# steineggerlab/folddisco

Measured on AMD Instinct MI355X. Metric: structures/sec indexed, higher is better.
Workload: dtype f32+u32; 1 GPU; Swiss-Prot scale: 542000 synthetic AFDB-shaped structures (175035960 residues, 17705019118 postings, 26085150307 value bytes) index build, PDBTrRosetta default; 1 rank(s), contiguous id ranges, per rank 1 build call(s) of <= 542000 structures: one resident index, no merge; structures=542000, structures_per_gpu=542000, residues=175035960, postings=17705019118, parallelism=shard-by-structure x1, build_calls_per_rank=1

## Files before the change

### folddisco_amd/csrc/fdgpu_api.hip

```cpp
#include <math.h>
#include <stdio.h>
#include <stdlib.h>
#include <string.h>
#include <algorithm>
#include <chrono>
#include <sys/mman.h>
#include <atomic>
#include <thread>
#include "fdgpu_internal.h"
#include <fcntl.h>
#include <unistd.h>
#include <cerrno>
#include <cstring>

#include "fd_api_common.h"
#include "fd_postings.h"

__global__ void k_uniq_flags(const uint32_t *__restrict__ keys, const uint32_t *__restrict__ ids, uint64_t n, uint8_t *__restrict__ flags) {
    uint64_t p = (uint64_t)blockIdx.x * blockDim.x + threadIdx.x;
    if (p < n) flags[p] = (p == 0 || keys[p] != keys[p - 1] || ids[p] != ids[p - 1]) ? 1 : 0;
}
__global__ void k_compact(const uint32_t *__restrict__ keys, const uint8_t *__restrict__ flags, const uint64_t *__restrict__ pos, uint64_t n,
                          uint32_t *__restrict__ out) {
    uint64_t p = (uint64_t)blockIdx.x * blockDim.x + threadIdx.x;
    if (p < n && flags[p]) out[pos[p]] = keys[p];
}
__global__ void k_gather_u64(const uint64_t *__restrict__ src, const uint64_t *__restrict__ idx, uint64_t n, uint64_t *__restrict__ dst) {
    uint64_t p = (uint64_t)blockIdx.x * blockDim.x + threadIdx.x;
    if (p < n) dst[p] = src[idx[p]];
}
void fd_launch_uniq_flags(const uint32_t *keys, const uint32_t *ids, uint64_t n, uint8_t *flags, hipStream_t st) {
    if (n) hipLaunchKernelGGL(k_uniq_flags, dim3((unsigned)((n + 255) / 256)), dim3(256), 0, st, keys, ids, n, flags);
}
void fd_launch_compact(const uint32_t *keys, const uint8_t *flags, const uint64_t *pos, uint64_t n, uint32_t *out, hipStream_t st) {
    if (n) hipLaunchKernelGGL(k_compact, dim3((unsigned)((n + 255) / 256)), dim3(256), 0, st, keys, flags, pos, n, out);
}
void fd_launch_gather_u64(const uint64_t *src, const uint64_t *idx, uint64_t n, uint64_t *dst, hipStream_t st) {
    if (n) hipLaunchKernelGGL(k_gather_u64, dim3((unsigned)((n + 255) / 256)), dim3(256), 0, st, src, idx, n, dst);
}

__global__ __launch_bounds__(256) void k_count_postings(const uint8_t *__restrict__ value, uint64_t n, unsigned long long *__restrict__ out) {
    unsigned long long acc = 0;
    for (uint64_t p = ((uint64_t)blockIdx.x * 256 + threadIdx.x) * 16; p < n; p += (uint64_t)gridDim.x * 256 * 16)
        for (uint64_t k = p; k < n && k < p + 16; ++k) acc += !(value[k] & 0x80u);
    for (int o = 32; o > 0; o >>= 1) acc += __shfl_down(acc, o);
    if ((threadIdx.x & 63) == 0 && acc) atomicAdd(out, acc);
}
hipError_t fd_count_postings(fdgpu_ctx *c, const uint8_t *value, uint64_t n, uint64_t *out) {
    unsigned long long np = 0;
    hipError_t e = hipSuccess;
    if (n) {
        e = c->ws[WS_TOTAL].ensure(64);
        if (e == hipSuccess) e = hipMemsetAsync(c->ws[WS_TOTAL].p, 0, 8, c->stream);
        if (e == hipSuccess) { hipLaunchKernelGGL(k_count_postings, dim3(2048), dim3(256), 0, c->stream, value, n, c->ws[WS_TOTAL].as<unsigned long long>()); e = hipGetLastError(); }
        if (e == hipSuccess) e = hipMemcpyAsync(&np, c->ws[WS_TOTAL].p, 8, hipMemcpyDeviceToHost, c->stream);
    }
    if (e == hipSuccess) e = hipStreamSynchronize(c->stream);
    *out = np;
    return e;
}

extern "C" const char *fdgpu_version(void) { return "folddisco_amd 0.1 (gfx950)"; }

static int fd_selfcheck(fdgpu_ctx *c) {
    const char *e = getenv("FDGPU_SELFCHECK");
    if (e && e[0] == '0') return FDGPU_OK;
    fd_hash_params p;
    memset(&p, 0, sizeof p);
    p.dist_cutoff = 20.0f; p.hash_type = FDGPU_HASH_PDBTR;
    const fd_hash_consts C = make_consts(&p);
    uint32_t *d = nullptr, h[24];
    HIPCHK(c, hipMalloc((void **)&d, sizeof h));
    fd_launch_selfcheck(C.q, d, c->stream);
    hipError_t he = hipGetLastError();
    if (he == hipSuccess) he = hipMemcpyAsync(h, d, sizeof h, hipMemcpyDeviceToHost, c->stream);
    if (he == hipSuccess) he = hipStreamSynchronize(c->stream);
    (void)hipFree(d);
    if (he != hipSuccess) { c->err = std::string("self-check launch: ") + hipGetErrorString(he); return FDGPU_EHIP; }
    static const uint32_t want[6] = {109329223u, 116878724u, 271858548u, 284511716u, 506948936u, 512052558u};
    for (int k = 0; k < 24; ++k)
        if (h[k] != want[k % 6]) {
            char b[256];
            snprintf(b, sizeof b, "self-check failed: 4CHA triad hash %d (%s evaluation) is %u, the reference's literal is %u (controller/graph.rs:71-79)", k % 6,
                     k < 6 ? "generic" : k < 12 ? "table" : k < 18 ? "speculative" : "speculative + squared-distance table", h[k], want[k % 6]);
            c->err = b;
            return FDGPU_EHIP;
        }
    int ok = 1;
    auto same = [](float a, float b) { uint32_t x, y; memcpy(&x, &a, 4); memcpy(&y, &b, 4); return x == y || (a != a && b != b); };
    for (int k = 1; k < FD_THETA_NSEG && ok; ++k) {
        float t;
        memcpy(&t, &fd_theta_thr_bits[k], 4);
        for (int u = -64; u <= 64 && ok; ++u) {
            uint32_t bits = fd_theta_thr_bits[k] + (uint32_t)u;
            float x;
            memcpy(&x, &bits, 4);
            if (!(x >= -1.0f && x <= 1.0f)) continue;
            const float a = acosf(x);
            ok = same(fd_acosf(x), a) && same(fd_sinf(a), sinf(a)) && same(fd_cosf(a), cosf(a));
        }
    }
    for (int m = 0; m < 4 && ok; ++m)
        for (int k = 1; k < FD_TOR_MAXSEG && ok; ++k)
            for (int u = -64; u <= 64 && ok; ++u) {
                uint32_t bits = fd_tor_thr_bits[m][k] + (uint32_t)u;
                float r;
                memcpy(&r, &bits, 4);
                if (!(r == r) || r > 3.0e38f) continue;
                const float y = (m & 1) ? -r : r, x = (m & 2) ? -1.0f : 1.0f;
                const float a = -atan2f(y, x);
                ok = same(-fd_atan2f(y, x), a) && same(fd_sinf(a), sinf(a)) && same(fd_cosf(a), cosf(a));
            }
    c->host_libm_matches = ok;
    if (!ok) {
        static bool warned = false;
        if (!warned) {
            warned = true;
            fprintf(stderr, "[fdgpu] warning: this host's libm (sinf/cosf/acosf/atan2f) differs from the glibc 2.35 generation the device arithmetic restates; a "
                            "reference build on this host can hash residue pairs at bin edges differently (rerun tools/gen_bin_tables.c + tools/check_libm.c)\n");
        }
    }
    return FDGPU_OK;
}
extern "C" int fdgpu_host_libm_matches(const fdgpu_ctx *c) { return c ? c->host_libm_matches : -1; }

static std::atomic<int> fd_live_contexts{0};
extern "C" void fdgpu_trim(void);
extern "C" int fdgpu_create(int device, fdgpu_ctx **out) {
    if (!out) return FDGPU_EINVAL;
    *out = nullptr;
    fdgpu_ctx *c = new (std::nothrow) fdgpu_ctx();
    if (!c) return FDGPU_ENOMEM;
    c->device = device;
    int n = 0;
    hipError_t e = hipGetDeviceCount(&n);
    if (e != hipSuccess || n <= 0 || device < 0 || device >= n) {
        c->err = e != hipSuccess ? std::string("hipGetDeviceCount: ") + hipGetErrorString(e) : "no such HIP device";
        *out = c;
        return FDGPU_EHIP;
    }
    if ((e = hipSetDevice(device)) != hipSuccess || (e = hipStreamCreate(&c->stream)) != hipSuccess) {
        c->err = std::string("hipSetDevice/hipStreamCreate: ") + hipGetErrorString(e);
        *out = c;
        return FDGPU_EHIP;
    }
    c->own_stream = true;
    c->counted = true;
    fd_live_contexts.fetch_add(1);
    if (hipMalloc((void **)&c->spec_miss, 8) == hipSuccess) (void)hipMemset(c->spec_miss, 0, 8);
    else c->spec_miss = nullptr;
    *out = c;
    return fd_selfcheck(c);
}
extern "C" int fdgpu_spec_fallbacks(fdgpu_ctx *c, uint64_t *out) { FD_LOCK(c);
    if (!c || !out) return FDGPU_EINVAL;
    *out = 0;
    if (!c->spec_miss) return FDGPU_OK;
    HIPCHK(c, hipStreamSynchronize(c->stream));
    HIPCHK(c, hipMemcpy(out, c->spec_miss, 8, hipMemcpyDeviceToHost));
    HIPCHK(c, hipMemset(c->spec_miss, 0, 8));
    return FDGPU_OK;
}
extern "C" void fdgpu_destroy(fdgpu_ctx *c) {
    if (!c) return;
    fd_lanes_destroy(c);
    if (c->spec_miss) (void)hipFree(c->spec_miss);
    for (auto &b : c->ws) b.release();
    for (auto &b : c->pool) (void)hipFree(b.p);
    for (auto e : c->event_pool) (void)hipEventDestroy(e);
    for (int k = 0; k < 16; ++k) { if (c->pin[k]) (void)hipHostFree(c->pin[k]); if (c->pin_ev[k]) (void)hipEventDestroy(c->pin_ev[k]); }
    for (int k = 0; k < 6; ++k) if (c->hbuf[k]) (void)hipHostFree(c->hbuf[k]);
    if (c->side_stream) (void)hipStreamDestroy(c->side_stream);
    if (c->own_stream && c->stream) (void)hipStreamDestroy(c->stream);
    const bool last = c->counted && fd_live_contexts.fetch_sub(1) == 1;
    delete c;
    if (last) fdgpu_trim();
}
extern "C" int fdgpu_release_workspaces(fdgpu_ctx *c) { FD_LOCK(c);
    if (!c) return FDGPU_EINVAL;
    HIPCHK(c, hipStreamSynchronize(c->stream));
    for (auto &b : c->ws) b.release();
    c->pool_drop();
    (void)hipGetLastError();
    return FDGPU_OK;
}
extern "C" int fdgpu_set_stream(fdgpu_ctx *c, void *s) { FD_LOCK(c);
    if (!c) return FDGPU_EINVAL;
    if (c->own_stream && c->stream) { (void)hipStreamSynchronize(c->stream); (void)hipStreamDestroy(c->stream); c->own_stream = false; }
    if (s) { c->stream = (hipStream_t)s; return FDGPU_OK; }
    HIPCHK(c, hipStreamCreate(&c->stream));
    c->own_stream = true;
    return FDGPU_OK;
}
extern "C" int fdgpu_synchronize(fdgpu_ctx *c) { FD_LOCK(c);
    if (!c) return FDGPU_EINVAL;
    HIPCHK(c, hipStreamSynchronize(c->stream));
    return FDGPU_OK;
}
extern "C" const char *fdgpu_last_error(const fdgpu_ctx *c) { return c ? c->err.c_str() : "null context"; }
#include <mutex>
#include <unordered_map>
namespace {
struct fd_out_blk { size_t cap; bool pinned; };
struct fd_out_pool {
    std::mutex mu;
    std::unordered_map<void *, fd_out_blk> live;
    std::vector<std::pair<fd_out_blk, void *>> idle;
    size_t idle_bytes = 0;
};
fd_out_pool &out_pool() { static fd_out_pool *p = new fd_out_pool(); return *p; }
const size_t FD_OUT_POOL_MIN = (size_t)64 << 10;
size_t fd_out_pool_cap() {
    static const size_t cap = [] { const char *e = getenv("FDGPU_OUT_POOL_MB"); return e ? (size_t)std::max(0L, atol(e)) << 20 : (size_t)256 << 20; }();
    return cap;
}
}
extern "C" void fdgpu_trim(void) {
    fd_out_pool &P = out_pool();
    std::vector<std::pair<fd_out_blk, void *>> drop;
    {
        std::lock_guard<std::mutex> lk(P.mu);
        drop.swap(P.idle);
        P.idle_bytes = 0;
    }
    for (auto &b : drop) { if (b.first.pinned) (void)hipHostFree(b.second); else free(b.second); }
}
void *fd_out_alloc(size_t bytes, bool pinned) {
    if (bytes < FD_OUT_POOL_MIN) return malloc(bytes ? bytes : 1);
    fd_out_pool &P = out_pool();
    {
        std::lock_guard<std::mutex> lk(P.mu);
        size_t best = (size_t)-1;
        for (size_t k = 0; k < P.idle.size(); ++k)
            if (P.idle[k].first.pinned == pinned && P.idle[k].first.cap >= bytes && P.idle[k].first.cap <= 2 * bytes + (1u << 20) &&
                (best == (size_t)-1 || P.idle[k].first.cap < P.idle[best].first.cap)) best = k;
        if (best != (size_t)-1) {
            void *p = P.idle[best].second;
            const fd_out_blk b = P.idle[best].first;
            P.idle.erase(P.idle.begin() + best);
            P.idle_bytes -= b.cap;
            P.live[p] = b;
            return p;
        }
    }
    const size_t cap = bytes + bytes / 4;
    void *p = nullptr;
    bool got_pinned = false;
    if (pinned && hipHostMalloc(&p, cap, hipHostMallocPortable) == hipSuccess && p) got_pinned = true;
    else { (void)hipGetLastError(); p = malloc(cap); }
    if (!p) return nullptr;
    std::lock_guard<std::mutex> lk(P.mu);
    P.live[p] = fd_out_blk{cap, got_pinned};
    return p;
}
extern "C" void fdgpu_free(void *p) {
    if (!p) return;
    fd_out_pool &P = out_pool();
    fd_out_blk b;
    {
        std::lock_guard<std::mutex> lk(P.mu);
        auto it = P.live.find(p);
        if (it == P.live.end()) { free(p); return; }
        b = it->second;
        P.live.erase(it);
        if (P.idle_bytes + b.cap <= fd_out_pool_cap()) { P.idle.emplace_back(b, p); P.idle_bytes += b.cap; return; }
    }
    if (b.pinned) (void)hipHostFree(p); else free(p);
}
extern "C" int fdgpu_enable_timing(fdgpu_ctx *c, int on) { FD_LOCK(c); if (!c) return FDGPU_EINVAL; c->timing = on != 0; return FDGPU_OK; }
extern "C" int fdgpu_last_timings(const fdgpu_ctx *c, const char **names, float *ms, uint64_t *bytes, int cap) { FD_LOCK(c);
    if (!c) return FDGPU_EINVAL;
    int n = 0;
    for (auto &t : c->timings) {
        if (n >= cap) break;
        float m = 0.f;
        if (hipEventElapsedTime(&m, t.ev0, t.ev1) != hipSuccess) m = -1.f;
        if (names) names[n] = t.name;
        if (ms) ms[n] = m;
        if (bytes) bytes[n] = t.bytes;
        ++n;
    }
    return n;
}

int fd_build_work_items(fdgpu_ctx *c, fdgpu_batch *b, bool with_hash_ok) {
    std::vector<uint32_t> ws, wi;
    std::vector<uint32_t> ro(b->n_struct + 1);
    for (uint64_t s = 0; s <= b->n_struct; ++s) ro[s] = (uint32_t)b->h_res_off[s];
    for (uint64_t s = 0; s < b->n_struct; ++s) {
        uint64_t R = b->h_res_off[s + 1] - b->h_res_off[s];
        if (R > 65535) FAIL(c, FDGPU_ERANGE, "structure with more than 65535 residues (reference max_residue, controller/mod.rs:40)");
        for (uint64_t t = 0; t < R; t += FD_WAVE) { ws.push_back((uint32_t)s); wi.push_back((uint32_t)(b->h_res_off[s] + t)); }
    }
    if (ws.size() > 0xfffffff0ull) FAIL(c, FDGPU_ERANGE, "too many tiles in one batch");
    b->n_work = (uint32_t)ws.size();
    HIPCHK(c, hipMalloc((void **)&b->res_off, ro.size() * 4));
    HIPCHK(c, hipMalloc((void **)&b->wi_struct, std::max<size_t>(ws.size(), 1) * 4));
    HIPCHK(c, hipMalloc((void **)&b->wi_i0, std::max<size_t>(wi.size(), 1) * 4));
    HIPCHK(c, hipMemcpyAsync(b->res_off, ro.data(), ro.size() * 4, hipMemcpyHostToDevice, c->stream));
    if (!ws.empty()) {
        HIPCHK(c, hipMemcpyAsync(b->wi_struct, ws.data(), ws.size() * 4, hipMemcpyHostToDevice, c->stream));
        HIPCHK(c, hipMemcpyAsync(b->wi_i0, wi.data(), wi.size() * 4, hipMemcpyHostToDevice, c->stream));
    }
    HIPCHK(c, hipMalloc((void **)&b->hash_ok, std::max<uint64_t>(b->n_res, 1)));
    if (with_hash_ok) fd_launch_hash_ok(b->aa, b->cb_valid, b->hash_ok, b->n_res, c->stream);
    HIPCHK(c, hipGetLastError());
    HIPCHK(c, hipStreamSynchronize(c->stream));
    return FDGPU_OK;
}

extern "C" int fdgpu_batch_upload(fdgpu_ctx *c, const fd_batch_desc *h, fdgpu_batch **out) { FD_LOCK(c);
    if (!c || !h || !out || !h->res_off || (h->n_struct && (!h->n_xyz || !h->ca_xyz || !h->cb_xyz || !h->aa))) return FDGPU_EINVAL;
    *out = nullptr;
    if (h->n_struct >= 0xffffffffull) FAIL(c, FDGPU_ERANGE, "too many structures in one batch");
    uint64_t R = h->res_off[h->n_struct];
    if (R >= 0xffffffffull) FAIL(c, FDGPU_ERANGE, "more than 2^32 residues in one batch");
    fdgpu_batch *b = new (std::nothrow) fdgpu_batch();
    if (!b) return FDGPU_ENOMEM;
    b->ctx = c; b->owns = true; b->n_struct = h->n_struct; b->n_res = R;
    b->h_res_off.assign(h->res_off, h->res_off + h->n_struct + 1);
    size_t rb = std::max<uint64_t>(R, 1);
    int rc = FDGPU_OK;
    auto up = [&](void **d, const void *src, size_t bytes) -> int {
        HIPCHK(c, hipMalloc(d, std::max<size_t>(bytes, 4)));
        if (bytes) HIPCHK(c, hipMemcpyAsync(*d, src, bytes, hipMemcpyHostToDevice, c->stream));
        return FDGPU_OK;
    };
    if ((rc = up((void **)&b->n_xyz, h->n_xyz, R * 12)) || (rc = up((void **)&b->ca_xyz, h->ca_xyz, R * 12)) ||
        (rc = up((void **)&b->cb_xyz, h->cb_xyz, R * 12)) || (rc = up((void **)&b->aa, h->aa, R))) { fdgpu_batch_destroy(b); return rc; }
    if (h->cb_valid && (rc = up((void **)&b->cb_valid, h->cb_valid, R))) { fdgpu_batch_destroy(b); return rc; }
    (void)rb;
    if ((rc = fd_build_work_items(c, b))) { fdgpu_batch_destroy(b); return rc; }
    *out = b;
    return FDGPU_OK;
}

extern "C" int fdgpu_batch_wrap_device(fdgpu_ctx *c, const fd_batch_desc *d, uint64_t total_residues, fdgpu_batch **out) { FD_LOCK(c);
    if (!c || !d || !out || !d->res_off) return FDGPU_EINVAL;
    *out = nullptr;
    fdgpu_batch *b = new (std::nothrow) fdgpu_batch();
    if (!b) return FDGPU_ENOMEM;
    b->ctx = c; b->owns = false; b->n_struct = d->n_struct; b->n_res = total_residues;
    b->n_xyz = (float *)d->n_xyz; b->ca_xyz = (float *)d->ca_xyz; b->cb_xyz = (float *)d->cb_xyz;
    b->aa = (uint8_t *)d->aa; b->cb_valid = (uint8_t *)d->cb_valid;
    b->h_res_off.resize(d->n_struct + 1);
    hipError_t e = hipMemcpy(b->h_res_off.data(), d->res_off, (d->n_struct + 1) * 8, hipMemcpyDeviceToHost);
    if (e != hipSuccess) { c->err = std::string("wrap_device: ") + hipGetErrorString(e); delete b; return FDGPU_EHIP; }
    if (b->h_res_off[d->n_struct] != total_residues) { c->err = "wrap_device: res_off[n] != total_residues"; delete b; return FDGPU_EINVAL; }
    int rc = fd_build_work_items(c, b);
    if (rc) { fdgpu_batch_destroy(b); return rc; }
    *out = b;
    return FDGPU_OK;
}

extern "C" void fdgpu_batch_destroy(fdgpu_batch *b) {
    if (!b) return;
    if (b->owns) { (void)hipFree(b->n_xyz); (void)hipFree(b->ca_xyz); (void)hipFree(b->cb_xyz); (void)hipFree(b->aa); (void)hipFree(b->cb_valid); }
    (void)hipFree(b->hash_ok); (void)hipFree(b->res_off); (void)hipFree(b->wi_struct); (void)hipFree(b->wi_i0);
    delete b;
}
extern "C" uint64_t fdgpu_batch_num_structures(const fdgpu_batch *b) { return b ? b->n_struct : 0; }
extern "C" uint64_t fdgpu_batch_num_residues(const fdgpu_batch *b) { return b ? b->n_res : 0; }

bool fd_hash_type_supported(uint32_t t) { return t <= 8u; }
fd_hash_consts make_consts_bins(const fd_hash_params *p, uint32_t nbd_req, uint32_t nba_req, bool either_zero_defaults) {
    const uint32_t type = p->hash_type;
    uint32_t cap_d = 16, def_d = 16, cap_a = 4, def_a = 4;
    if (type == FD_HASH_PDBMOTIF) { cap_d = 32; def_d = 18; cap_a = 32; def_a = 9; }
    else if (type == FD_HASH_PDBMOTIF_SINCOS) { cap_d = 16; def_d = 8; cap_a = 16; def_a = 3; }
    else if (type == FD_HASH_FD_ANGLE) { cap_d = 8; def_d = 8; cap_a = 32; def_a = 32; }
    else if (type == FD_HASH_FD_DIST) { cap_d = 32; def_d = 32; cap_a = 16; def_a = 16; }
    else if (type == FD_HASH_TRROSETTA) { cap_d = 8; def_d = 8; cap_a = 4; def_a = 3; }
    else if (type == FD_HASH_PPF || type == FD_HASH_TERTIARY) { cap_d = 16; def_d = 8; cap_a = 8; def_a = 3; }
    else if (type == FD_HASH_HYBRID) { cap_d = 16; def_d = 16; cap_a = 4; def_a = 4; }
    const bool dflt = either_zero_defaults && (nbd_req == 0 || nba_req == 0);
    float nd = (dflt || nbd_req == 0) ? (float)def_d : (nbd_req > cap_d ? (float)cap_d : (float)nbd_req);
    float na = (dflt || nba_req == 0) ? (float)def_a : (nba_req > cap_a ? (float)cap_a : (float)nba_req);
    fd_hash_consts C;
    C.seg_mul = 1; C.seg_cfg = 0;
    const float PI_F = 3.14159274f;
    float a_min = -1.0f, a_max = 1.0f;
    if (type == FD_HASH_PDBMOTIF) { a_min = 0.0f; a_max = 180.0f; }
    else if (type == FD_HASH_FD_ANGLE || type == FD_HASH_FD_DIST) { a_min = -PI_F; a_max = PI_F; }
    volatile float cont_d = (20.0f - 2.0f) / (nd - 1.0f);
    volatile float cont_a = (a_max - a_min) / (na - 1.0f);
    float n180 = type == FD_HASH_FD_ANGLE ? fminf(na, 32.0f) : fminf(na, 8.0f);
    volatile float cont_t = (PI_F - 0.0f) / (n180 - 1.0f);
    C.q.dist_disc = 1.0f / cont_d;
    C.q.ang_disc = 1.0f / cont_a;
    C.q.ang2_disc = 1.0f / cont_t;
    C.q.type = type;
    float cut = p->dist_cutoff;
    float d2 = cut * cut;
    while (sqrtf(d2) > cut) d2 = nextafterf(d2, 0.0f);
    while (sqrtf(nextafterf(d2, INFINITY)) <= cut) d2 = nextafterf(d2, INFINITY);
    C.d2_max = d2;
    const char *ex = getenv("FDGPU_EXACT");
    const bool exact_only = ex && ex[0] == '1';
    C.use_tab = (type == FD_HASH_PDBTR && na == 4.0f) ? (exact_only ? 1 : 2) : 0;
    const char *dt = getenv("FDGPU_DTAB");
    if (C.use_tab == 2 && nd == 16.0f && !(dt && dt[0] == '0')) C.use_tab = 3;
    C.spec_miss = nullptr;
    return C;
}

fd_hash_consts make_consts(const fd_hash_params *p) { return make_consts_bins(p, p->nbin_dist, p->nbin_angle, true); }
fd_hash_consts fd_make_consts(const fd_hash_params *p) { return make_consts(p); }
uint32_t fd_num_bin_configs(const fd_hash_params *p) { return p->n_multiple_bins ? p->n_multiple_bins : 1u; }
fd_hash_consts fd_make_consts_cfg(const fd_hash_params *p, uint32_t k) {
    if (!p->n_multiple_bins) return make_consts(p);
    return make_consts_bins(p, p->multiple_bins[k][0], p->multiple_bins[k][1], false);
}
bool fd_multiple_bins_valid(const fd_hash_params *p) {
    if (p->n_multiple_bins > FDGPU_MAX_MULTIPLE_BINS) return false;
    for (uint32_t k = 0; k < p->n_multiple_bins; ++k)
        if (p->multiple_bins[k][0] == 0 || p->multiple_bins[k][1] == 0) return false;
    return true;
}

int d2h_u64(fdgpu_ctx *c, const uint64_t *dev, uint64_t *host) {
    HIPCHK(c, hipMemcpyAsync(host, dev, 8, hipMemcpyDeviceToHost, c->stream));
    HIPCHK(c, hipStreamSynchronize(c->stream));
    return FDGPU_OK;
}

static int count_and_scan(fdgpu_ctx *c, const fdgpu_batch *b, const fd_hash_consts &C, uint64_t *P, bool unordered = false) {
    uint64_t S = b->n_struct;
    HIPCHK(c, c->ws[WS_COUNTS].ensure((S + 1) * 4));
    HIPCHK(c, c->ws[WS_CURSOR].ensure((S + 1) * 4));
    HIPCHK(c, c->ws[WS_SEGOFF].ensure((S + 2) * 8));
    HIPCHK(c, c->ws[WS_SCANTMP].ensure(fd_scan_tmp_elems(std::max<uint64_t>(S, b->n_res)) * 8 + 64));
    HIPCHK(c, c->ws[WS_TOTAL].ensure(64));
    HIPCHK(c, hipMemsetAsync(c->ws[WS_COUNTS].p, 0, (S + 1) * 4, c->stream));
    HIPCHK(c, hipMemsetAsync(c->ws[WS_CURSOR].p, 0, (S + 1) * 4, c->stream));
    {
        StageTimer t(c, "pair_count", b->n_res * 13);
        if (unordered) fd_launch_pair_count2(b->view(), C, c->ws[WS_COUNTS].as<uint32_t>(), c->stream);
        else fd_launch_pair_count(b->view(), C, c->ws[WS_COUNTS].as<uint32_t>(), c->stream);
    }
    {
        StageTimer t(c, "segment_scan", S * 12);
        fd_exclusive_scan<uint32_t>(c->ws[WS_COUNTS].as<uint32_t>(), S, c->ws[WS_SEGOFF].as<uint64_t>(), c->ws[WS_SCANTMP].as<uint64_t>(),
                                    c->ws[WS_TOTAL].as<uint64_t>(), c->stream);
    }
    HIPCHK(c, hipGetLastError());
    return d2h_u64(c, c->ws[WS_TOTAL].as<uint64_t>(), P);
}

static int ensure_sort_ws(fdgpu_ctx *c, uint64_t P, size_t id_bytes = 4) {
    size_t kb = std::max<uint64_t>(P, 1) * 4, ib = std::max<uint64_t>(P, 1) * id_bytes + 16;
    if (kb > c->ws[WS_KEYS_A].cap + ((size_t)1 << 30) || kb > c->ws[WS_KEYS_B].cap + ((size_t)1 << 30)) c->pool_drop();
    HIPCHK(c, c->ws[WS_KEYS_A].ensure(kb));
    HIPCHK(c, c->ws[WS_IDS_A].ensure(ib));
    HIPCHK(c, c->ws[WS_KEYS_B].ensure(kb));
    HIPCHK(c, c->ws[WS_IDS_B].ensure(ib));
    HIPCHK(c, c->ws[WS_GHIST].ensure((size_t)256 * std::max<uint32_t>(fd_rs_num_tiles(P), 1) * 4));
    HIPCHK(c, c->ws[WS_TOT].ensure((256 + (size_t)(fd_rs_num_tiles(P) / 128 + 2) * 256) * 8));
    return FDGPU_OK;
}

int sort_pairs(fdgpu_ctx *c, uint32_t *ka, uint32_t *va, uint32_t *kb, uint32_t *vb, uint64_t n, int key_bits) {
    return fd_radix_sort_pairs(ka, va, kb, vb, n, key_bits, c->ws[WS_GHIST].as<uint32_t>(), c->ws[WS_TOT].as<uint64_t>(), c->stream, c);
}

extern "C" int fdgpu_hash_batch(fdgpu_ctx *c, const fdgpu_batch *b, const fd_hash_params *p, int sort_dedup, uint32_t **hashes,
                                uint64_t **hash_off) { FD_LOCK(c);
    if (!c || !b || !p || !hashes || !hash_off) return FDGPU_EINVAL;
    *hashes = nullptr; *hash_off = nullptr;
    if (p->n_multiple_bins) FAIL(c, FDGPU_EINVAL, "hash_batch: multiple_bins is honoured by the index build and the query calls only");
    if (!fd_hash_type_supported(p->hash_type)) FAIL(c, FDGPU_EINVAL, "hash_type: only the encodings over the (d_CA, d_CB, theta, tau1, tau2) descriptor are built (0, 1, 3, 7, 8)");
    reset_timings(c);
    fd_hash_consts C = make_consts(p);
    uint64_t S = b->n_struct, R = b->n_res;
    uint64_t *h_off = (uint64_t *)malloc((S + 1) * 8);
    if (!h_off) return FDGPU_ENOMEM;
    hipStream_t st = c->stream;
    if (!sort_dedup) {
        HIPCHK(c, c->ws[WS_MISC0].ensure((R + 1) * 4));
        HIPCHK(c, c->ws[WS_MISC1].ensure((R + 2) * 8));
        HIPCHK(c, c->ws[WS_SCANTMP].ensure(fd_scan_tmp_elems(std::max<uint64_t>(S, R)) * 8 + 64));
        HIPCHK(c, c->ws[WS_TOTAL].ensure(64));
        HIPCHK(c, hipMemsetAsync(c->ws[WS_MISC0].p, 0, (R + 1) * 4, st));
        fd_launch_row_count(b->view(), C, c->ws[WS_MISC0].as<uint32_t>(), p->dist_cutoff, st);
        fd_exclusive_scan<uint32_t>(c->ws[WS_MISC0].as<uint32_t>(), R, c->ws[WS_MISC1].as<uint64_t>(), c->ws[WS_SCANTMP].as<uint64_t>(),
                                    c->ws[WS_TOTAL].as<uint64_t>(), st);
        HIPCHK(c, hipGetLastError());
        uint64_t P = 0;
        int rc = d2h_u64(c, c->ws[WS_TOTAL].as<uint64_t>(), &P);
        if (rc) { free(h_off); return rc; }
        HIPCHK(c, c->ws[WS_KEYS_A].ensure(std::max<uint64_t>(P, 1) * 4));
        fd_launch_row_emit(b->view(), C, c->ws[WS_MISC1].as<uint64_t>(), c->ws[WS_KEYS_A].as<uint32_t>(), p->dist_cutoff, nullptr, 0u, st);
        HIPCHK(c, hipGetLastError());
        uint32_t *h = (uint32_t *)malloc(std::max<uint64_t>(P, 1) * 4);
        std::vector<uint64_t> row_off(R + 1);
        if (!h) { free(h_off); return FDGPU_ENOMEM; }
        HIPCHK(c, hipMemcpyAsync(h, c->ws[WS_KEYS_A].p, P * 4, hipMemcpyDeviceToHost, st));
        HIPCHK(c, hipMemcpyAsync(row_off.data(), c->ws[WS_MISC1].p, (R + 1) * 8, hipMemcpyDeviceToHost, st));
        HIPCHK(c, hipStreamSynchronize(st));
        for (uint64_t s = 0; s <= S; ++s) h_off[s] = row_off[b->h_res_off[s]];
        *hashes = h; *hash_off = h_off;
        return FDGPU_OK;
    }
    if (fd_own_descriptor(p->hash_type)) { free(h_off); FAIL(c, FDGPU_EINVAL, "hash_batch: this encoding is served in the reference's raw order only (sort_dedup = 0)"); }
    uint64_t P = 0;
    int rc = count_and_scan(c, b, C, &P);
    if (rc) { free(h_off); return rc; }
    if (P >= 0xffffffffull) { free(h_off); FAIL(c, FDGPU_ERANGE, "more than 2^32 residue pairs in one batch; split the batch"); }
    if ((rc = ensure_sort_ws(c, P))) { free(h_off); return rc; }
    uint32_t *ka = c->ws[WS_KEYS_A].as<uint32_t>(), *ia = c->ws[WS_IDS_A].as<uint32_t>();
    uint32_t *kb = c->ws[WS_KEYS_B].as<uint32_t>(), *ib = c->ws[WS_IDS_B].as<uint32_t>();
    fd_launch_pair_emit(b->view(), C, c->ws[WS_SEGOFF].as<uint64_t>(), c->ws[WS_CURSOR].as<uint32_t>(), ka, ia, 0u, st);
    int cur = sort_pairs(c, ka, ia, kb, ib, P, 32);
    uint32_t *k1 = cur ? kb : ka, *i1 = cur ? ib : ia, *k2 = cur ? ka : kb, *i2 = cur ? ia : ib;
    int id_bits = 1;
    while (id_bits < 32 && (1ull << id_bits) < std::max<uint64_t>(S, 2)) ++id_bits;
    int cur2 = sort_pairs(c, i1, k1, i2, k2, P, id_bits);
    uint32_t *ids_s = cur2 ? i2 : i1, *keys_s = cur2 ? k2 : k1, *spare = cur2 ? k1 : k2;
    HIPCHK(c, c->ws[WS_MISC0].ensure(std::max<uint64_t>(P, 1)));
    HIPCHK(c, c->ws[WS_MISC1].ensure((P + 2) * 8));
    HIPCHK(c, c->ws[WS_SCANTMP].ensure(fd_scan_tmp_elems(std::max<uint64_t>(P, S)) * 8 + 64));
    fd_launch_uniq_flags(keys_s, ids_s, P, c->ws[WS_MISC0].as<uint8_t>(), st);
    fd_exclusive_scan<uint8_t>(c->ws[WS_MISC0].as<uint8_t>(), P, c->ws[WS_MISC1].as<uint64_t>(), c->ws[WS_SCANTMP].as<uint64_t>(),
                               c->ws[WS_TOTAL].as<uint64_t>(), st);
    fd_launch_compact(keys_s, c->ws[WS_MISC0].as<uint8_t>(), c->ws[WS_MISC1].as<uint64_t>(), P, spare, st);
    HIPCHK(c, c->ws[WS_MISC2].ensure((S + 2) * 8));
    fd_launch_gather_u64(c->ws[WS_MISC1].as<uint64_t>(), c->ws[WS_SEGOFF].as<uint64_t>(), S + 1, c->ws[WS_MISC2].as<uint64_t>(), st);
    HIPCHK(c, hipGetLastError());
    uint64_t U = 0;
    if ((rc = d2h_u64(c, c->ws[WS_TOTAL].as<uint64_t>(), &U))) { free(h_off); return rc; }
    uint32_t *h = (uint32_t *)malloc(std::max<uint64_t>(U, 1) * 4);
    if (!h) { free(h_off); return FDGPU_ENOMEM; }
    HIPCHK(c, hipMemcpyAsync(h, spare, U * 4, hipMemcpyDeviceToHost, st));
    HIPCHK(c, hipMemcpyAsync(h_off, c->ws[WS_MISC2].p, (S + 1) * 8, hipMemcpyDeviceToHost, st));
    HIPCHK(c, hipStreamSynchronize(st));
    *hashes = h; *hash_off = h_off;
    return FDGPU_OK;
}

extern "C" int fdgpu_hash_batch_rows(fdgpu_ctx *c, const fdgpu_batch *b, const fd_hash_params *p, uint32_t **hashes, uint32_t **partner, uint64_t **row_off) { FD_LOCK(c);
    if (!c || !b || !p || !hashes || !partner || !row_off) return FDGPU_EINVAL;
    *hashes = nullptr; *partner = nullptr; *row_off = nullptr;
    if (p->n_multiple_bins) FAIL(c, FDGPU_EINVAL, "hash_batch_rows: multiple_bins is honoured by the index build and the query calls only");
    if (!fd_hash_type_supported(p->hash_type)) FAIL(c, FDGPU_EINVAL, "hash_type: unknown encoding");
    reset_timings(c);
    const fd_hash_consts C = make_consts(p);
    const uint64_t R = b->n_res;
    hipStream_t st = c->stream;
    HIPCHK(c, c->ws[WS_MISC0].ensure((R + 1) * 4));
    HIPCHK(c, c->ws[WS_MISC1].ensure((R + 2) * 8));
    HIPCHK(c, c->ws[WS_SCANTMP].ensure(fd_scan_tmp_elems(std::max<uint64_t>(b->n_struct, R)) * 8 + 64));
    HIPCHK(c, c->ws[WS_TOTAL].ensure(64));
    HIPCHK(c, hipMemsetAsync(c->ws[WS_MISC0].p, 0, (R + 1) * 4, st));
    fd_launch_row_count(b->view(), C, c->ws[WS_MISC0].as<uint32_t>(), p->dist_cutoff, st);
    fd_exclusive_scan<uint32_t>(c->ws[WS_MISC0].as<uint32_t>(), R, c->ws[WS_MISC1].as<uint64_t>(), c->ws[WS_SCANTMP].as<uint64_t>(),
                                c->ws[WS_TOTAL].as<uint64_t>(), st);
    HIPCHK(c, hipGetLastError());
    uint64_t P = 0;
    int rc = d2h_u64(c, c->ws[WS_TOTAL].as<uint64_t>(), &P);
    if (rc) return rc;
    HIPCHK(c, c->ws[WS_KEYS_A].ensure(std::max<uint64_t>(P, 1) * 4));
    HIPCHK(c, c->ws[WS_IDS_A].ensure(std::max<uint64_t>(P, 1) * 4));
    fd_launch_row_emit(b->view(), C, c->ws[WS_MISC1].as<uint64_t>(), c->ws[WS_KEYS_A].as<uint32_t>(), p->dist_cutoff, c->ws[WS_IDS_A].as<uint32_t>(), 0u, st, 1);
    HIPCHK(c, hipGetLastError());
    uint32_t *h = (uint32_t *)malloc(std::max<uint64_t>(P, 1) * 4), *pj = (uint32_t *)malloc(std::max<uint64_t>(P, 1) * 4);
    uint64_t *ro = (uint64_t *)malloc((R + 1) * 8);
    if (!h || !pj || !ro) { free(h); free(pj); free(ro); return FDGPU_ENOMEM; }
    hipError_t e = hipMemcpyAsync(h, c->ws[WS_KEYS_A].p, P * 4, hipMemcpyDeviceToHost, st);
    if (e == hipSuccess) e = hipMemcpyAsync(pj, c->ws[WS_IDS_A].p, P * 4, hipMemcpyDeviceToHost, st);
    if (e == hipSuccess) e = hipMemcpyAsync(ro, c->ws[WS_MISC1].p, (R + 1) * 8, hipMemcpyDeviceToHost, st);
    if (e == hipSuccess) e = hipStreamSynchronize(st);
    if (e != hipSuccess) { free(h); free(pj); free(ro); c->err = std::string("hash_batch_rows: ") + hipGetErrorString(e); return FDGPU_EHIP; }
    *hashes = h; *partner = pj; *row_off = ro;
    return FDGPU_OK;
}

hipError_t fd_index_block(fdgpu_ctx *pool, size_t bytes, void **p, size_t *cap) {
    if (!pool) return hipMalloc(p, bytes);
    hipError_t e;
    *p = pool->pool_alloc(bytes, &e);
    *cap = pool->last_cap;
    return e;
}
int fd_index_new(fdgpu_ctx *c, bool pooled, uint64_t H, uint64_t value_len, bool with_last, fdgpu_index **out) {
    *out = nullptr;
    fdgpu_index *ix = new (std::nothrow) fdgpu_index();
    if (!ix) FAIL(c, FDGPU_ENOMEM, "index alloc: out of memory");
    ix->ctx = pooled ? c : nullptr; ix->n_hashes = H;
    hipError_t e = hipSuccess;
    if (value_len != FD_VALUE_LATER) { ix->value_len = value_len; e = fd_index_block(ix->ctx, value_len + FD_VALUE_SLACK, (void **)&ix->value, &ix->cap_value); }
    if (e == hipSuccess) e = fd_index_block(ix->ctx, std::max<uint64_t>(H, 1) * 4, (void **)&ix->hashes, &ix->cap_hashes);
    if (e == hipSuccess) e = fd_index_block(ix->ctx, (H + 1) * 8, (void **)&ix->offsets, &ix->cap_offsets);
    if (e == hipSuccess && with_last) e = fd_index_block(ix->ctx, std::max<uint64_t>(H, 1) * 4, (void **)&ix->last_ids, &ix->cap_last);
    if (e != hipSuccess) { c->err = std::string("index alloc: ") + hipGetErrorString(e); fdgpu_index_destroy(ix); return FDGPU_EHIP; }
    *out = ix;
    return FDGPU_OK;
}
__global__ void k_ix_order(const uint8_t *__restrict__ sel, const uint8_t *__restrict__ is_long, const uint64_t *__restrict__ sel_pre,
                           const uint64_t *__restrict__ long_pre, uint64_t H, uint32_t *__restrict__ order, uint32_t *__restrict__ place) {
    const uint64_t t = (uint64_t)blockIdx.x * blockDim.x + threadIdx.x;
    if (t >= H || (sel && !sel[t])) return;
    const uint64_t n_long = long_pre[H];
    const uint64_t g = is_long[t] ? long_pre[t] : n_long + ((sel ? sel_pre[t] : t) - long_pre[t]);
    order[g] = (uint32_t)t;
    if (place) place[t] = (uint32_t)g;
}
void fd_order_long_first(const uint8_t *sel, const uint8_t *is_long, uint64_t H, uint64_t *sel_pre, uint64_t *long_pre, uint64_t *scan_tmp,
                         uint64_t *total_dev, uint32_t *order, uint32_t *place, hipStream_t st) {
    if (sel) fd_exclusive_scan<uint8_t>(sel, H, sel_pre, scan_tmp, total_dev, st);
    fd_exclusive_scan<uint8_t>(is_long, H, long_pre, scan_tmp, total_dev, st);
    hipLaunchKernelGGL(k_ix_order, dim3(fd_grid(H, 256)), dim3(256), 0, st, sel, is_long, sel_pre, long_pre, H, order, place);
}
extern "C" void fdgpu_index_destroy(fdgpu_index *ix) {
    if (!ix) return;
    FD_LOCK(ix->ctx);
    if (ix->ctx) {
        ix->ctx->pool_free(ix->hashes, ix->cap_hashes); ix->ctx->pool_free(ix->offsets, ix->cap_offsets); ix->ctx->pool_free(ix->value, ix->cap_value);
    } else { (void)hipFree(ix->hashes); (void)hipFree(ix->offsets); (void)hipFree(ix->value); }
    if (ix->ctx && ix->cap_last) ix->ctx->pool_free(ix->last_ids, ix->cap_last);
    else (void)hipFree(ix->last_ids);
    if (ix->penalty) (void)hipFree(ix->penalty);
    if (ix->lens) (void)hipFree(ix->lens);
    if (ix->ck_meta) (void)hipFree(ix->ck_meta);
    if (ix->ck_ent) (void)hipFree(ix->ck_ent);
    delete ix;
}
extern "C" int fdgpu_index_set_first_id(fdgpu_index *ix, uint64_t first_id) { if (!ix || first_id + ix->n_structures > 0xffffffffull) return FDGPU_EINVAL; ix->first_id = first_id; return FDGPU_OK; }
extern "C" uint64_t fdgpu_index_num_hashes(const fdgpu_index *ix) { return ix ? ix->n_hashes : 0; }
extern "C" uint64_t fdgpu_index_value_len(const fdgpu_index *ix) { return ix ? ix->value_len : 0; }
extern "C" uint64_t fdgpu_index_num_postings(const fdgpu_index *ix) { return ix ? ix->n_postings : 0; }
extern "C" uint64_t fdgpu_index_num_structures(const fdgpu_index *ix) { return ix ? ix->n_structures : 0; }

#define FDGPU_RETRY_WIDE 1000
static int encode_sorted_stream(fdgpu_ctx *c, const uint32_t *ks, const void *is, int codec, uint64_t first_id, uint64_t P, uint64_t S, fdgpu_index **out) {
    hipStream_t st = c->stream;
    const bool el6 = codec != 0;
    int rc;
    uint32_t nt = std::max<uint32_t>(fd_enc_num_tiles(P), 1);
    HIPCHK(c, c->ws[WS_TILE_B].ensure((size_t)(nt + 1) * 4));
    HIPCHK(c, c->ws[WS_TILE_H].ensure((size_t)(nt + 1) * 4));
    HIPCHK(c, c->ws[WS_TILE_P].ensure((size_t)(nt + 1) * 4));
    HIPCHK(c, c->ws[WS_TILE_BO].ensure((size_t)(nt + 2) * 8));
    HIPCHK(c, c->ws[WS_TILE_HO].ensure((size_t)(nt + 2) * 8));
    HIPCHK(c, c->ws[WS_TILE_PO].ensure((size_t)(nt + 2) * 8));
    HIPCHK(c, c->ws[WS_SCANTMP].ensure(fd_scan_tmp_elems(std::max<uint64_t>(nt, S)) * 8 + 64));
    uint64_t tot[5] = {0, 0, 0, 0, 0};
    uint64_t nt_eff = P ? fd_enc_num_tiles(P) : 0;
    {
        StageTimer t(c, "encode_sizes", P * (el6 ? 6 : 8));
        HIPCHK(c, hipMemsetAsync(c->ws[WS_TILE_B].p, 0, (size_t)(nt + 1) * 4, st));
        HIPCHK(c, hipMemsetAsync(c->ws[WS_TILE_H].p, 0, (size_t)(nt + 1) * 4, st));
        HIPCHK(c, hipMemsetAsync(c->ws[WS_TILE_P].p, 0, (size_t)(nt + 1) * 4, st));
        fd_launch_enc_sizes(ks, is, codec, (uint32_t)first_id, P, c->ws[WS_TILE_B].as<uint32_t>(), c->ws[WS_TILE_H].as<uint32_t>(), c->ws[WS_TILE_P].as<uint32_t>(),
                            c->ws[WS_SEGOFF].as<uint64_t>(), S, c->ws[WS_MISC3].as<uint64_t>() + 8, st);
        uint64_t *totd = c->ws[WS_MISC3].as<uint64_t>();
        fd_exclusive_scan<uint32_t>(c->ws[WS_TILE_B].as<uint32_t>(), nt_eff, c->ws[WS_TILE_BO].as<uint64_t>(), c->ws[WS_SCANTMP].as<uint64_t>(), totd + 0, st);
        fd_exclusive_scan<uint32_t>(c->ws[WS_TILE_H].as<uint32_t>(), nt_eff, c->ws[WS_TILE_HO].as<uint64_t>(), c->ws[WS_SCANTMP].as<uint64_t>(), totd + 1, st);
        fd_exclusive_scan<uint32_t>(c->ws[WS_TILE_P].as<uint32_t>(), nt_eff, c->ws[WS_TILE_PO].as<uint64_t>(), c->ws[WS_SCANTMP].as<uint64_t>(), totd + 2, st);
    }
    HIPCHK(c, hipGetLastError());
    HIPCHK(c, hipMemcpyAsync(tot, c->ws[WS_MISC3].p, 40, hipMemcpyDeviceToHost, st));
    HIPCHK(c, hipStreamSynchronize(st));
    if (tot[4]) FAIL(c, FDGPU_ERANGE, "index build: one (residue-pair bucket, key digit) group holds 2^32 keys or more; build the shard in several calls and merge");
    if (el6 && tot[3]) return FDGPU_RETRY_WIDE;
    fdgpu_index *ix = nullptr;
    if ((rc = fd_index_new(c, true, tot[1], tot[0], true, &ix))) return rc;
    ix->n_postings = tot[2]; ix->n_structures = S; ix->first_id = first_id;
    {
        StageTimer t(c, "encode_write", P * (el6 ? 6 : 8) + ix->value_len + ix->n_hashes * 12);
        fd_launch_enc_write(ks, is, codec, (uint32_t)first_id, P, c->ws[WS_TILE_BO].as<uint64_t>(), c->ws[WS_TILE_HO].as<uint64_t>(), ix->value, ix->hashes, ix->offsets,
                            ix->last_ids, c->ws[WS_MISC3].as<uint64_t>(), ix->n_hashes, c->ws[WS_MISC3].as<uint64_t>() + 8, st);
    }
    const hipError_t e = hipGetLastError();
    if (e != hipSuccess) { c->err = std::string("encode launch: ") + hipGetErrorString(e); fdgpu_index_destroy(ix); return FDGPU_EHIP; }
    *out = ix;
    return FDGPU_OK;
}

static int index_build_impl(fdgpu_ctx *c, const fdgpu_batch *b, const fd_hash_params *p, uint64_t first_id, fdgpu_index **out, bool force32) {
    if (!c || !b || !p || !out) return FDGPU_EINVAL;
    *out = nullptr;
    if (!fd_hash_type_supported(p->hash_type)) FAIL(c, FDGPU_EINVAL, "hash_type: only the encodings over the (d_CA, d_CB, theta, tau1, tau2) descriptor are built (0, 1, 3, 7, 8)");
    reset_timings(c);
    if (first_id + b->n_struct > 0xffffffffull) FAIL(c, FDGPU_ERANGE, "structure ids exceed 32 bits");
    if (!fd_multiple_bins_valid(p)) FAIL(c, FDGPU_EINVAL, "multiple_bins: at most 8 (dist, angle) bin pairs, no zero counts");
    const uint32_t n_cfg = fd_num_bin_configs(p);
    fd_hash_consts C = fd_make_consts_cfg(p, 0);
    C.spec_miss = c->spec_miss;
    hipStream_t st = c->stream;
    uint64_t S = b->n_struct, P = 0;
    HIPCHK(c, c->ws[WS_FRAMES].ensure(std::max<uint64_t>(b->n_res, 1) * sizeof(fd_frame)));
    const bool own = fd_own_descriptor(p->hash_type);
    if (own && n_cfg > 1) FAIL(c, FDGPU_EINVAL, "multiple_bins is built for the encodings over the PDBTrRosetta descriptor only");
    const bool ids16 = !own && !force32 && S <= (1ull << 18);
    const bool msd_env = [] { const char *e = getenv("FDGPU_MSD"); return !(e && e[0] == '0'); }();
    const bool msd = msd_env && !own && !force32 && S <= (1ull << 24) && n_cfg == 1 && p->hash_type == FDGPU_HASH_PDBTR && S > 0;
    const bool el6 = ids16 || msd;
    const int codec = msd ? 2 : ids16 ? 1 : 0;
    const uint32_t NB = 40;
    fd_batch_view V = b->view();
    HIPCHK(c, c->ws[WS_MISC3].ensure(512));
    HIPCHK(c, hipMemsetAsync(c->ws[WS_MISC3].p, 0, 64, st));
    C.wide_flag = c->ws[WS_MISC3].as<unsigned long long>() + 3;
    if (msd) {
        HIPCHK(c, c->ws[WS_CA_PERM].ensure(std::max<uint64_t>(b->n_res, 1) * 12));
        HIPCHK(c, c->ws[WS_OK_PERM].ensure(std::max<uint64_t>(b->n_res, 1)));
        HIPCHK(c, c->ws[WS_AA_PERM].ensure(std::max<uint64_t>(b->n_res, 1)));
        StageTimer t(c, "frames", b->n_res * (37 + sizeof(fd_frame) + 14));
        fd_launch_frames_perm(V, c->ws[WS_FRAMES].p, c->ws[WS_CA_PERM].as<float>(), c->ws[WS_OK_PERM].as<uint8_t>(), c->ws[WS_AA_PERM].as<uint8_t>(), C.wide_flag, st);
        V.ca_xyz = c->ws[WS_CA_PERM].as<float>(); V.hash_ok = c->ws[WS_OK_PERM].as<uint8_t>(); V.aa = c->ws[WS_AA_PERM].as<uint8_t>();
        V.n_xyz = nullptr; V.cb_xyz = nullptr;
    } else {
        StageTimer t(c, "frames", b->n_res * (37 + sizeof(fd_frame)));
        fd_launch_frames(b->view(), b->n_res, c->ws[WS_FRAMES].p, st);
    }
    uint64_t P1 = 0;
    int rc;
    if (own) {
        const uint64_t R = b->n_res;
        HIPCHK(c, c->ws[WS_MISC0].ensure((R + 1) * 4));
        HIPCHK(c, c->ws[WS_MISC1].ensure((R + 2) * 8));
        HIPCHK(c, c->ws[WS_SCANTMP].ensure(fd_scan_tmp_elems(std::max<uint64_t>(R, S)) * 8 + 64));
        HIPCHK(c, c->ws[WS_TOTAL].ensure(64));
        HIPCHK(c, hipMemsetAsync(c->ws[WS_MISC0].p, 0, (R + 1) * 4, st));
        {
            StageTimer t(c, "pair_count", R * 37);
            fd_launch_row_count(b->view(), C, c->ws[WS_MISC0].as<uint32_t>(), p->dist_cutoff, st);
            fd_exclusive_scan<uint32_t>(c->ws[WS_MISC0].as<uint32_t>(), R, c->ws[WS_MISC1].as<uint64_t>(), c->ws[WS_SCANTMP].as<uint64_t>(),
                                        c->ws[WS_TOTAL].as<uint64_t>(), st);
        }
        HIPCHK(c, hipGetLastError());
        rc = d2h_u64(c, c->ws[WS_TOTAL].as<uint64_t>(), &P1);
    } else if (msd) {
        const uint64_t NS = NB * S;
        HIPCHK(c, c->ws[WS_COUNTS].ensure((NS + 1) * 4));
        HIPCHK(c, c->ws[WS_CURSOR].ensure((NS + 1) * 4));
        HIPCHK(c, c->ws[WS_SEGOFF].ensure((NS + 2) * 8));
        HIPCHK(c, c->ws[WS_SCANTMP].ensure(fd_scan_tmp_elems(std::max<uint64_t>(NS, b->n_res)) * 8 + 64));
        HIPCHK(c, c->ws[WS_TOTAL].ensure(64));
        HIPCHK(c, hipMemsetAsync(c->ws[WS_COUNTS].p, 0, (NS + 1) * 4, st));
        HIPCHK(c, hipMemsetAsync(c->ws[WS_CURSOR].p, 0, (NS + 1) * 4, st));
        {
            StageTimer t(c, "pair_count", b->n_res * 14);
            fd_launch_pair_count_msd(V, C, c->ws[WS_COUNTS].as<uint32_t>(), st);
        }
        {
            StageTimer t(c, "segment_scan", NS * 12);
            fd_exclusive_scan<uint32_t>(c->ws[WS_COUNTS].as<uint32_t>(), NS, c->ws[WS_SEGOFF].as<uint64_t>(), c->ws[WS_SCANTMP].as<uint64_t>(),
                                        c->ws[WS_TOTAL].as<uint64_t>(), st);
        }
        HIPCHK(c, hipGetLastError());
        rc = d2h_u64(c, c->ws[WS_TOTAL].as<uint64_t>(), &P1);
        uint64_t odd = 0;
        if (!rc) rc = d2h_u64(c, (const uint64_t *)C.wide_flag, &odd);
        if (!rc && odd) return FDGPU_RETRY_WIDE;
    } else {
        rc = count_and_scan(c, b, C, &P1, true);
    }
    if (rc) return rc;
    P = P1 * n_cfg;
    if (P >= 0xffffffffull && !msd) FAIL(c, FDGPU_ERANGE, "more than 2^32 residue pairs in one build call; split the shard");
    if (P >= (1ull << 35)) FAIL(c, FDGPU_ERANGE, "more than 2^35 residue pairs in one build call; split the shard");
    if ((rc = ensure_sort_ws(c, P, el6 ? 2 : 4))) return rc;
    uint32_t *ka = c->ws[WS_KEYS_A].as<uint32_t>(), *kb = c->ws[WS_KEYS_B].as<uint32_t>();
    void *ia = c->ws[WS_IDS_A].p, *ib = c->ws[WS_IDS_B].p;
    {
        StageTimer t(c, "pair_emit", b->n_res * 37 + P * (el6 ? 6 : 8));
        if (own) fd_launch_row_emit(b->view(), C, c->ws[WS_MISC1].as<uint64_t>(), ka, p->dist_cutoff, (uint32_t *)ia, (uint32_t)first_id, st);
        else if (msd) fd_launch_pair_emit_msd(V, c->ws[WS_FRAMES].p, C, c->ws[WS_SEGOFF].as<uint64_t>(), c->ws[WS_CURSOR].as<uint32_t>(), ka, (uint16_t *)ia, st);
        else for (uint32_t k = 0; k < n_cfg; ++k) {
            fd_hash_consts Ck = fd_make_consts_cfg(p, k);
            Ck.spec_miss = C.spec_miss; Ck.wide_flag = C.wide_flag; Ck.seg_mul = n_cfg; Ck.seg_cfg = k;
            if (k) HIPCHK(c, hipMemsetAsync(c->ws[WS_CURSOR].p, 0, (S + 1) * 4, st));
            fd_launch_pair_emit2(b->view(), c->ws[WS_FRAMES].p, Ck, c->ws[WS_SEGOFF].as<uint64_t>(), c->ws[WS_CURSOR].as<uint32_t>(), ka, ia, ids16,
                                 (uint32_t)first_id, st);
        }
    }
    int cur;
    if (msd) {
        static const fd_rs_digit digits[3] = {{0, 24}, {1, 0}, {1, 8}};
        HIPCHK(c, c->ws[WS_GHIST].ensure((size_t)256 * fd_rs_seg_num_tiles(P, NB) * 4));
        HIPCHK(c, c->ws[WS_TOT].ensure(fd_rs_seg_tot_words(P, NB) * 8));
        HIPCHK(c, c->ws[WS_SEG_TAB].ensure(fd_rs_seg_tab_bytes(P, NB)));
        cur = fd_radix_sort_pairs16_seg(ka, (uint16_t *)ia, kb, (uint16_t *)ib, P, c->ws[WS_SEGOFF].as<uint64_t>(), S, NB, digits, 3, c->ws[WS_GHIST].as<uint32_t>(),
                                        c->ws[WS_TOT].as<uint64_t>(), c->ws[WS_SEG_TAB].p, st, c, c->ws[WS_MISC3].as<unsigned long long>() + 4);
    } else if (ids16) cur = fd_radix_sort_pairs16(ka, (uint16_t *)ia, kb, (uint16_t *)ib, P, 32, c->ws[WS_GHIST].as<uint32_t>(), c->ws[WS_TOT].as<uint64_t>(), st, c);
    else cur = sort_pairs(c, ka, (uint32_t *)ia, kb, (uint32_t *)ib, P, 32);
    const uint32_t *ks = cur ? kb : ka;
    const void *is = cur ? ib : ia;
    return encode_sorted_stream(c, ks, is, codec, first_id, P, S, out);
}

extern "C" int fdgpu_index_build(fdgpu_ctx *c, const fdgpu_batch *b, const fd_hash_params *p, uint64_t first_id, fdgpu_index **out) { FD_LOCK(c);
    const char *e32 = getenv("FDGPU_IDS32");
    int rc = index_build_impl(c, b, p, first_id, out, e32 && e32[0] == '1');
    if (rc == FDGPU_RETRY_WIDE) rc = index_build_impl(c, b, p, first_id, out, true);
    return rc;
}

extern "C" int fdgpu_debug_encode_stream(fdgpu_ctx *c, const uint32_t *hashes, const uint32_t *ids, uint64_t n, fdgpu_index **out) { FD_LOCK(c);
    if (!c || !out || (n && (!hashes || !ids))) return FDGPU_EINVAL;
    *out = nullptr;
    if (n >= 0xffffffffull) FAIL(c, FDGPU_ERANGE, "encode_stream: 2^32 elements or more");
    uint64_t S = 0;
    for (uint64_t p = 0; p < n; ++p) {
        if (p && (hashes[p - 1] > hashes[p] || (hashes[p - 1] == hashes[p] && ids[p - 1] > ids[p]))) FAIL(c, FDGPU_EINVAL, "encode_stream: the stream is not sorted by (hash, id)");
        S = std::max<uint64_t>(S, (uint64_t)ids[p] + 1);
    }
    reset_timings(c);
    hipStream_t st = c->stream;
    HIPCHK(c, c->ws[WS_MISC3].ensure(512));
    HIPCHK(c, hipMemsetAsync(c->ws[WS_MISC3].p, 0, 64, st));
    HIPCHK(c, c->ws[WS_KEYS_A].ensure(std::max<uint64_t>(n, 1) * 4));
    HIPCHK(c, c->ws[WS_IDS_A].ensure(std::max<uint64_t>(n, 1) * 4));
    if (n) {
        HIPCHK(c, hipMemcpyAsync(c->ws[WS_KEYS_A].p, hashes, n * 4, hipMemcpyHostToDevice, st));
        HIPCHK(c, hipMemcpyAsync(c->ws[WS_IDS_A].p, ids, n * 4, hipMemcpyHostToDevice, st));
    }
    return encode_sorted_stream(c, c->ws[WS_KEYS_A].as<uint32_t>(), c->ws[WS_IDS_A].p, 0, 0, n, S, out);
}

#define FD_PIN_SLOTS 16
#define FD_PIN_BYTES ((size_t)16 << 20)
hipError_t fd_d2h_big(fdgpu_ctx *c, void *dst, const void *src, size_t bytes) {
    if (bytes < 4 * FD_PIN_BYTES) return bytes ? hipMemcpyAsync(dst, src, bytes, hipMemcpyDeviceToHost, c->stream) : hipSuccess;
    for (int k = 0; k < FD_PIN_SLOTS; ++k) {
        hipError_t e = hipSuccess;
        if (!c->pin[k]) e = hipHostMalloc(&c->pin[k], FD_PIN_BYTES, hipHostMallocDefault);
        if (e == hipSuccess && !c->pin_ev[k]) e = hipEventCreateWithFlags(&c->pin_ev[k], hipEventDisableTiming);
        if (e != hipSuccess) return hipMemcpyAsync(dst, src, bytes, hipMemcpyDeviceToHost, c->stream);
    }
    {
        const uintptr_t a = ((uintptr_t)dst + 0x1fffff) & ~(uintptr_t)0x1fffff, b = ((uintptr_t)dst + bytes) & ~(uintptr_t)0x1fffff;
        if (b > a) (void)madvise((void *)a, b - a, MADV_HUGEPAGE);
    }
    const size_t n_chunks = (bytes + FD_PIN_BYTES - 1) / FD_PIN_BYTES;
    std::vector<std::thread> drain(FD_PIN_SLOTS);
    hipError_t err = hipSuccess;
    const int dev = c->device;
    for (size_t i = 0; i < n_chunks && err == hipSuccess; ++i) {
        const int k = (int)(i % FD_PIN_SLOTS);
        if (drain[k].joinable()) drain[k].join();
        const size_t off = i * FD_PIN_BYTES, n = std::min(FD_PIN_BYTES, bytes - off);
        err = hipMemcpyAsync(c->pin[k], (const uint8_t *)src + off, n, hipMemcpyDeviceToHost, c->stream);
        if (err == hipSuccess) err = hipEventRecord(c->pin_ev[k], c->stream);
        if (err != hipSuccess) break;
        void *pin = c->pin[k];
        hipEvent_t ev = c->pin_ev[k];
        drain[k] = std::thread([=]() { (void)hipSetDevice(dev); (void)hipEventSynchronize(ev); memcpy((uint8_t *)dst + off, pin, n); });
    }
    for (auto &t : drain) if (t.joinable()) t.join();
    return err;
}

extern "C" int fdgpu_index_export(fdgpu_ctx *c, const fdgpu_index *ix, uint8_t **value, uint64_t *value_len, uint32_t **hashes,
                                  uint64_t **offsets, uint64_t *n_hashes) { FD_LOCK(c);
    if (!c || !ix || !value || !value_len || !hashes || !offsets || !n_hashes) return FDGPU_EINVAL;
    uint8_t *v = (uint8_t *)malloc(std::max<uint64_t>(ix->value_len, 1));
    uint32_t *h = (uint32_t *)malloc(std::max<uint64_t>(ix->n_hashes, 1) * 4);
    uint64_t *o = (uint64_t *)malloc((ix->n_hashes + 1) * 8);
    if (!v || !h || !o) { free(v); free(h); free(o); return FDGPU_ENOMEM; }
    hipError_t e = fd_d2h_big(c, v, ix->value, ix->value_len);
    if (e == hipSuccess) e = fd_d2h_big(c, h, ix->hashes, ix->n_hashes * 4);
    if (e == hipSuccess) e = fd_d2h_big(c, o, ix->offsets, (ix->n_hashes + 1) * 8);
    if (e == hipSuccess) e = hipStreamSynchronize(c->stream);
    if (e != hipSuccess) { free(v); free(h); free(o); c->err = std::string("index export: ") + hipGetErrorString(e); return FDGPU_EHIP; }
    *value = v; *value_len = ix->value_len; *hashes = h; *offsets = o; *n_hashes = ix->n_hashes;
    return FDGPU_OK;
}

extern "C" int fdgpu_index_load(fdgpu_ctx *c, const uint32_t *hashes, const uint64_t *offsets, uint64_t H, const uint8_t *value,
                                uint64_t vlen, uint64_t n_structures, fdgpu_index **out) { FD_LOCK(c);
    if (!c || !out || (H && (!hashes || !offsets)) || (vlen && !value)) return FDGPU_EINVAL;
    *out = nullptr;
    fdgpu_index *ix = nullptr;
    int rc = fd_index_new(c, false, H, vlen, false, &ix);
    if (rc) return rc;
    ix->n_structures = n_structures;
    hipError_t e = hipSuccess;
    uint64_t zero = 0;
    if ((vlen && (e = hipMemcpyAsync(ix->value, value, vlen, hipMemcpyHostToDevice, c->stream)) != hipSuccess) ||
        (H && (e = hipMemcpyAsync(ix->hashes, hashes, H * 4, hipMemcpyHostToDevice, c->stream)) != hipSuccess) ||
        (e = hipMemcpyAsync(ix->offsets, H ? offsets : &zero, (H + 1) * 8, hipMemcpyHostToDevice, c->stream)) != hipSuccess ||
        (e = hipStreamSynchronize(c->stream)) != hipSuccess) {
        c->err = std::string("index load: ") + hipGetErrorString(e);
        fdgpu_index_destroy(ix);
        return FDGPU_EHIP;
    }
    if ((e = fd_count_postings(c, ix->value, vlen, &ix->n_postings)) != hipSuccess) {
        (void)hipGetLastError();
        c->err = std::string("index load: counting the postings: ") + hipGetErrorString(e);
        fdgpu_index_destroy(ix);
        return FDGPU_EHIP;
    }
    *out = ix;
    return FDGPU_OK;
}

hipError_t fd_d2h_to_file(fdgpu_ctx *c, int fd, uint64_t file_off, const void *src, size_t bytes, std::atomic<int> *io_err) {
    if (!bytes) return hipSuccess;
    for (int k = 0; k < FD_PIN_SLOTS; ++k) {
        hipError_t e = hipSuccess;
        if (!c->pin[k]) e = hipHostMalloc(&c->pin[k], FD_PIN_BYTES, hipHostMallocDefault);
        if (e == hipSuccess && !c->pin_ev[k]) e = hipEventCreateWithFlags(&c->pin_ev[k], hipEventDisableTiming);
        if (e != hipSuccess) return e;
    }
    const size_t n_chunks = (bytes + FD_PIN_BYTES - 1) / FD_PIN_BYTES;
    std::vector<std::thread> drain(FD_PIN_SLOTS);
    hipError_t err = hipSuccess;
    const int dev = c->device;
    for (size_t i = 0; i < n_chunks && err == hipSuccess; ++i) {
        const int k = (int)(i % FD_PIN_SLOTS);
        if (drain[k].joinable()) drain[k].join();
        const size_t off = i * FD_PIN_BYTES, n = std::min(FD_PIN_BYTES, bytes - off);
        err = hipMemcpyAsync(c->pin[k], (const uint8_t *)src + off, n, hipMemcpyDeviceToHost, c->stream);
        if (err == hipSuccess) err = hipEventRecord(c->pin_ev[k], c->stream);
        if (err != hipSuccess) break;
        const uint8_t *pin = (const uint8_t *)c->pin[k];
        hipEvent_t ev = c->pin_ev[k];
        drain[k] = std::thread([=]() {
            (void)hipSetDevice(dev);
            if (hipEventSynchronize(ev) != hipSuccess) { int z = 0; io_err->compare_exchange_strong(z, EIO); return; }
            size_t done = 0;
            while (done < n) {
                const ssize_t w = pwrite(fd, pin + done, n - done, (off_t)(file_off + off + done));
                if (w < 0) { if (errno == EINTR) continue; int z = 0; io_err->compare_exchange_strong(z, errno ? errno : EIO); return; }
                done += (size_t)w;
            }
        });
    }
    for (auto &t : drain) if (t.joinable()) t.join();
    return err;
}

extern "C" int fdgpu_reserve_staging(fdgpu_ctx *c) { FD_LOCK(c);
    if (!c) return FDGPU_EINVAL;
    for (int k = 0; k < FD_PIN_SLOTS; ++k) {
        if (!c->pin[k]) HIPCHK(c, hipHostMalloc(&c->pin[k], FD_PIN_BYTES, hipHostMallocDefault));
        if (!c->pin_ev[k]) HIPCHK(c, hipEventCreateWithFlags(&c->pin_ev[k], hipEventDisableTiming));
    }
    return FDGPU_OK;
}

extern "C" int fdgpu_index_save(fdgpu_ctx *c, const fdgpu_index *ix, const char *prefix) { FD_LOCK(c);
    if (!c || !ix || !prefix) return FDGPU_EINVAL;
    const std::string p(prefix);
    const uint64_t H = ix->n_hashes;
    std::atomic<int> io_err{0};
    hipError_t e = hipSuccess;
    const int fv = open(p.c_str(), O_WRONLY | O_CREAT | O_TRUNC, 0644);
    const int fo = fv >= 0 ? open((p + ".offset").c_str(), O_WRONLY | O_CREAT | O_TRUNC, 0644) : -1;
    if (fv < 0 || fo < 0) { if (fv >= 0) close(fv); FAIL(c, FDGPU_EINVAL, "index save: cannot write " + p); }
    if (pwrite(fo, &H, 8, 0) != 8) io_err = errno ? errno : EIO;
    const bool trace = getenv("FDGPU_TRACE") != nullptr;
    const auto t0 = std::chrono::steady_clock::now();
    auto ms = [&]() { return std::chrono::duration<double, std::milli>(std::chrono::steady_clock::now() - t0).count(); };
    if (trace) {
        for (int k = 0; k < FD_PIN_SLOTS && e == hipSuccess; ++k) if (!c->pin[k]) e = hipHostMalloc(&c->pin[k], FD_PIN_BYTES, hipHostMallocDefault);
        fprintf(stderr, "[index_save] staging slots page-locked at %.3f ms\n", ms());
    }
    if (e == hipSuccess) e = fd_d2h_to_file(c, fv, 0, ix->value, ix->value_len, &io_err);
    if (trace) fprintf(stderr, "[index_save] %llu value bytes streamed at %.3f ms\n", (unsigned long long)ix->value_len, ms());
    if (e == hipSuccess) e = fd_d2h_to_file(c, fo, 8, ix->hashes, H * 4, &io_err);
    if (e == hipSuccess) e = fd_d2h_to_file(c, fo, 8 + H * 4, ix->offsets, (H + 1) * 8, &io_err);
    if (e == hipSuccess) e = hipStreamSynchronize(c->stream);
    if (trace) fprintf(stderr, "[index_save] offset file streamed at %.3f ms\n", ms());
    if (close(fv) != 0 && !io_err) io_err = errno ? errno : EIO;
    if (close(fo) != 0 && !io_err) io_err = errno ? errno : EIO;
    if (trace) fprintf(stderr, "[index_save] files closed at %.3f ms\n", ms());
    if (e != hipSuccess) { c->err = std::string("index save: ") + hipGetErrorString(e); return FDGPU_EHIP; }
    if (io_err) FAIL(c, FDGPU_EINVAL, "index save: cannot write " + p + " (" + strerror(io_err) + ")");
    return FDGPU_OK;
}

__global__ void k_debug_libm(int op, const float *__restrict__ a, const float *__restrict__ b, float *__restrict__ out, uint64_t n) {
    uint64_t k = (uint64_t)blockIdx.x * blockDim.x + threadIdx.x;
    if (k >= n) return;
    float x = a[k], s, c;
    switch (op) {
        case 0: fdd_sincosf(x, &s, &c); out[k] = s; break;
        case 1: fdd_sincosf(x, &s, &c); out[k] = c; break;
        case 2: out[k] = fdd_acosf(x); break;
        case 3: out[k] = fdd_atanf(x); break;
        default: out[k] = fdd_atan2f(x, b[k]); break;
    }
}
extern "C" int fdgpu_debug_libm(fdgpu_ctx *c, int op, const float *a, const float *b, float *out, uint64_t n) { FD_LOCK(c);
    if (!c || !a || !out || (op == 4 && !b) || op < 0 || op > 4) return FDGPU_EINVAL;
    if (!n) return FDGPU_OK;
    hipStream_t st = c->stream;
    HIPCHK(c, c->ws[WS_MISC0].ensure(n * 4));
    HIPCHK(c, c->ws[WS_MISC1].ensure(n * 4));
    HIPCHK(c, c->ws[WS_MISC2].ensure(n * 4));
    HIPCHK(c, hipMemcpyAsync(c->ws[WS_MISC0].p, a, n * 4, hipMemcpyHostToDevice, st));
    if (b) HIPCHK(c, hipMemcpyAsync(c->ws[WS_MISC1].p, b, n * 4, hipMemcpyHostToDevice, st));
    hipLaunchKernelGGL(k_debug_libm, dim3((unsigned)((n + 255) / 256)), dim3(256), 0, st, op, c->ws[WS_MISC0].as<float>(),
                       c->ws[WS_MISC1].as<float>(), c->ws[WS_MISC2].as<float>(), n);
    HIPCHK(c, hipGetLastError());
    HIPCHK(c, hipMemcpyAsync(out, c->ws[WS_MISC2].p, n * 4, hipMemcpyDeviceToHost, st));
    HIPCHK(c, hipStreamSynchronize(st));
    return FDGPU_OK;
}
```

### folddisco_amd/csrc/fdgpu_internal.h

```cpp
#pragma once
#include <hip/hip_runtime.h>
#include <stdint.h>
#include <functional>
#include <mutex>
#include <string>
#include <vector>
#include "../../include/fdgpu.h"
#include "../../include/fdgpu_debug.h"
#include "fd_device.h"
#include "fd_geom_other.h"
#include "fd_retrieve_host.h"

#include <condition_variable>
#include <thread>
struct fd_host_pool {
    std::vector<std::thread> th;
    std::mutex mu;
    std::condition_variable cv, cv_done;
    const std::function<void()> *job = nullptr;
    uint64_t gen = 0;
    unsigned want = 0, taken = 0, active = 0;
    bool stop = false;
    void loop() {
        uint64_t seen = 0;
        for (;;) {
            const std::function<void()> *f = nullptr;
            {
                std::unique_lock<std::mutex> lk(mu);
                cv.wait(lk, [&] { return stop || (gen != seen && taken < want); });
                if (stop) return;
                seen = gen; ++taken; f = job;
            }
            (*f)();
            {
                std::lock_guard<std::mutex> lk(mu);
                --active;
            }
            cv_done.notify_one();
        }
    }
    void run(unsigned n, const std::function<void()> &f) {
        if (n <= 1) { f(); return; }
        const unsigned helpers = n - 1;
        {
            std::lock_guard<std::mutex> lk(mu);
            while (th.size() < helpers) th.emplace_back([this] { loop(); });
            job = &f; want = helpers; taken = 0; active = helpers; ++gen;
        }
        cv.notify_all();
        f();
        std::unique_lock<std::mutex> lk(mu);
        cv_done.wait(lk, [&] { return active == 0; });
        job = nullptr;
    }
    ~fd_host_pool() {
        {
            std::lock_guard<std::mutex> lk(mu);
            stop = true;
        }
        cv.notify_all();
        for (auto &t : th) t.join();
    }
};

struct fd_devbuf {
    void *p = nullptr;
    size_t cap = 0;
    hipError_t ensure(size_t bytes) {
        if (bytes <= cap) return hipSuccess;
        size_t want = bytes + (bytes < ((size_t)4 << 30) ? bytes / 16 : (size_t)0) + 256;
        if (cap && cap < (64u << 20) && want < cap + cap / 2) want = cap + cap / 2;
        if (p) { hipError_t e = hipFree(p); p = nullptr; cap = 0; if (e != hipSuccess) return e; }
        hipError_t e = hipMalloc(&p, want);
        if (e != hipSuccess) { p = nullptr; return e; }
        cap = want;
        return hipSuccess;
    }
    void release() { if (p) (void)hipFree(p); p = nullptr; cap = 0; }
    template <typename T> T *as() const { return reinterpret_cast<T *>(p); }
};

struct fd_timing_entry { const char *name; hipEvent_t ev0, ev1; uint64_t bytes; };

enum {
    WS_COUNTS, WS_CURSOR, WS_SEGOFF, WS_SCANTMP, WS_TOTAL, WS_KEYS_A, WS_IDS_A, WS_KEYS_B, WS_IDS_B, WS_GHIST, WS_TOT,
    WS_TILE_B, WS_TILE_H, WS_TILE_P, WS_TILE_BO, WS_TILE_HO , WS_TILE_PO, WS_MISC0, WS_MISC1, WS_MISC2, WS_MISC3, WS_MISC4, WS_MISC5, WS_FRAMES,
    WS_CQ_KIDX, WS_CQ_NSEG, WS_CQ_WSTART, WS_CQ_SEGSUM, WS_CQ_TOPN,
    WS_QT_RANGES, WS_QT_COMPACT, WS_QT_COUNT, WS_QT_AUX, WS_RS_PLAN, WS_RS_REC, WS_RS_RECRES, WS_QT_PARTIAL, WS_QT_SURV, WS_QT_ROWBITS, WS_QT_STREAM, WS_QT_STAB, WS_QT_PIECEP, WS_QT_WIN, WS_QT_HEAD, WS_RS_SPLIT, WS_MP_QSET,
    WS_CA_PERM, WS_OK_PERM, WS_AA_PERM, WS_SEG_TAB,
    WS_RS_TAB, WS_RS_SEG, WS_RS_OUT, WS_RS_RES, WS_RS_KX, WS_RS_KY, WS_RS_KOFF, WS_RS_SOL, WS_RS_CNT, WS_RS_GQ, WS_MP_ACT, WS_MP_Q,
    WS_SG_TAB , WS_SG_TAB_B, WS_SG_PAIRS, WS_SG_CURSOR,
    WS_SG_NB_PART , WS_SG_NB_OUT ,
    WS_COUNT
};

struct fdgpu_ctx {
    int device = 0;
    hipStream_t stream = nullptr;
    bool own_stream = false;
    std::string err;
    uint32_t last_retrieve_path = 0;
    uint32_t last_count_path = 0;
    fd_devbuf ws[WS_COUNT];
    bool timing = false;
    mutable std::recursive_mutex mu;
    int host_libm_matches = -1;
    unsigned long long *spec_miss = nullptr;
    std::vector<fd_timing_entry> timings;
    std::vector<hipEvent_t> event_pool;
    size_t event_used = 0;
    hipStream_t side_stream = nullptr;
    void *hbuf[6] = {nullptr, nullptr, nullptr, nullptr, nullptr, nullptr};
    size_t hbuf_cap[6] = {0, 0, 0, 0, 0, 0};
    void *host_pinned(int k, size_t bytes) {
        if (hbuf_cap[k] >= bytes) return hbuf[k];
        if (hbuf[k]) (void)hipHostFree(hbuf[k]);
        hbuf[k] = nullptr; hbuf_cap[k] = 0;
        const size_t want = bytes + bytes / 4 + 4096;
        if (hipHostMalloc(&hbuf[k], want, hipHostMallocDefault) != hipSuccess) { hbuf[k] = nullptr; return nullptr; }
        hbuf_cap[k] = want;
        return hbuf[k];
    }
    void *pin[16] = {};
    hipEvent_t pin_ev[16] = {};
    struct pooled { void *p; size_t cap; };
    std::vector<pooled> pool;
    void *pool_alloc(size_t bytes, hipError_t *err) {
        *err = hipSuccess;
        size_t best = (size_t)-1;
        for (size_t k = 0; k < pool.size(); ++k)
            if (pool[k].cap >= bytes && pool[k].cap <= bytes + bytes / 4 + 4096 && (best == (size_t)-1 || pool[k].cap < pool[best].cap)) best = k;
        if (best != (size_t)-1) { void *p = pool[best].p; last_cap = pool[best].cap; pool.erase(pool.begin() + best); return p; }
        void *p = nullptr;
        size_t want = bytes + bytes / 32 + 256;
        *err = hipMalloc(&p, want);
        if (*err != hipSuccess) {
            pool_drop();
            (void)hipGetLastError();
            *err = hipMalloc(&p, want);
            if (*err != hipSuccess) return nullptr;
        }
        last_cap = want;
        return p;
    }
    void pool_drop() { for (auto &b : pool) (void)hipFree(b.p); pool.clear(); }
    void pool_free(void *p, size_t cap) {
        if (!p) return;
        if (pool.size() >= 96) { (void)hipFree(p); return; }
        pool.push_back({p, cap});
    }
    size_t last_cap = 0;
    bool counted = false;
    const void *mp_bintab_at = nullptr; size_t mp_bintab_cap = 0;
    fd_host_pool host_pool;
    bool is_lane = false;
    unsigned small_par(unsigned n) const { return is_lane ? 1u : std::min(n, std::max(1u, std::thread::hardware_concurrency())); }
    void *lanes = nullptr;
};
void fd_lanes_destroy(fdgpu_ctx *c);

static inline hipEvent_t fd_next_event(fdgpu_ctx *c) {
    if (c->event_used == c->event_pool.size()) {
        hipEvent_t e;
        if (hipEventCreate(&e) != hipSuccess) return nullptr;
        c->event_pool.push_back(e);
    }
    return c->event_pool[c->event_used++];
}
struct StageTimer {
    fdgpu_ctx *c;
    size_t idx = (size_t)-1;
    StageTimer(fdgpu_ctx *ctx, const char *name, uint64_t bytes) : c(ctx) {
        if (!c || !c->timing) return;
        fd_timing_entry t;
        t.name = name; t.bytes = bytes; t.ev0 = fd_next_event(c); t.ev1 = fd_next_event(c);
        if (!t.ev0 || !t.ev1) return;
        (void)hipEventRecord(t.ev0, c->stream);
        c->timings.push_back(t);
        idx = c->timings.size() - 1;
    }
    ~StageTimer() { if (idx != (size_t)-1) (void)hipEventRecord(c->timings[idx].ev1, c->stream); }
};

#define FD_LOCK(c) std::unique_lock<std::recursive_mutex> _fd_lk; if (c) { _fd_lk = std::unique_lock<std::recursive_mutex>((c)->mu); (void)hipSetDevice((c)->device); }

struct fdgpu_batch {
    fdgpu_ctx *ctx = nullptr;
    bool owns = false;
    uint64_t n_struct = 0, n_res = 0;
    uint32_t n_work = 0;
    float *n_xyz = nullptr, *ca_xyz = nullptr, *cb_xyz = nullptr;
    uint8_t *aa = nullptr, *cb_valid = nullptr, *hash_ok = nullptr;
    uint32_t *res_off = nullptr, *wi_struct = nullptr, *wi_i0 = nullptr;
    std::vector<uint64_t> h_res_off;
    fd_batch_view view() const {
        fd_batch_view v;
        v.n_xyz = n_xyz; v.ca_xyz = ca_xyz; v.cb_xyz = cb_xyz; v.aa = aa; v.hash_ok = hash_ok; v.res_off = res_off;
        v.wi_struct = wi_struct; v.wi_i0 = wi_i0; v.n_struct = (uint32_t)n_struct; v.n_work = n_work;
        return v;
    }
};

int fd_build_work_items(fdgpu_ctx *c, fdgpu_batch *b, bool with_hash_ok = true);

#include <atomic>
static inline uint64_t fd_next_index_uid() { static std::atomic<uint64_t> n{1}; return n.fetch_add(1); }
struct fdgpu_index {
    fdgpu_ctx *ctx = nullptr;
    uint64_t n_hashes = 0, value_len = 0, n_postings = 0, n_structures = 0, first_id = 0;
    uint32_t *hashes = nullptr;
    uint64_t *offsets = nullptr;
    uint8_t *value = nullptr;
    mutable uint32_t *last_ids = nullptr;
    size_t cap_hashes = 0, cap_offsets = 0, cap_value = 0, cap_last = 0;
    mutable uint32_t *lens = nullptr;
    mutable std::mutex lens_mu;
    uint64_t uid = fd_next_index_uid();
    float *penalty = nullptr;
    mutable unsigned long long *ck_meta = nullptr;
    mutable void *ck_ent = nullptr;
    mutable uint64_t ck_n = 0, ck_first = 0, ck_S = 0;
    mutable bool ck_failed = false;
    mutable uint32_t ck_fail_skips = 0;
};

#define FD_VALUE_LATER (~0ull)
int fd_index_new(fdgpu_ctx *c, bool pooled, uint64_t H, uint64_t value_len, bool with_last, fdgpu_index **out);
hipError_t fd_index_block(fdgpu_ctx *pool, size_t bytes, void **p, size_t *cap);
int fd_index_last_ids(fdgpu_ctx *c, const fdgpu_index *ix);
hipError_t fd_count_postings(fdgpu_ctx *c, const uint8_t *value, uint64_t n, uint64_t *out);
static inline unsigned fd_grid(uint64_t n, uint64_t per) { return (unsigned)((n + per - 1) / per); }

#define FD_IXERR_DAMAGED 1u
#define FD_IXERR_LONG 2u
#define FD_LONG_LIST_BYTES 16384u
void fd_order_long_first(const uint8_t *sel, const uint8_t *is_long, uint64_t H, uint64_t *sel_pre, uint64_t *long_pre, uint64_t *scan_tmp,
                         uint64_t *total_dev, uint32_t *order, uint32_t *place, hipStream_t st);
static inline int fd_index_last_ids_staged(fdgpu_ctx *c, const fdgpu_index *ix, const char *stage) {
    if (ix->last_ids || !ix->n_hashes) return FDGPU_OK;
    StageTimer t(c, stage, ix->value_len + ix->n_hashes * 12);
    return fd_index_last_ids(c, ix);
}
struct fd_rows_dev { const uint32_t *val; const uint64_t *row_off; uint64_t n; };
int fd_rows_device(fdgpu_ctx *c, const fdgpu_index *ix, uint64_t id_lo, uint64_t id_hi, const char *what, fd_rows_dev *out);
static inline int fd_index_op_failed(fdgpu_ctx *c, int rc, fdgpu_index *const *made, size_t n = 1) {
    (void)hipStreamSynchronize(c->stream);
    for (size_t k = 0; k < n; ++k) fdgpu_index_destroy(made[k]);
    return rc;
}

struct fd_cq_dev_out {
    bool got = false, overflow = false; const void *recs = nullptr; const void *state = nullptr; uint32_t top_n = 0, cap = 0;
    std::vector<uint32_t> counts;
    const std::function<void()> *while_running = nullptr;
    uint32_t head_n = 0;
    const fd_count_rec *head = nullptr;
};
int fd_count_query_batch_impl(fdgpu_ctx *c, const fdgpu_index *ix, uint64_t n_queries, const uint64_t *q_off, const uint32_t *q_hash,
                              const uint32_t *q_node, const uint32_t *q_edge_j, const float *q_idf, const float *penalty, uint32_t top_n,
                              fd_count_rec **out, uint64_t **out_off, bool allow_dense, fd_cq_dev_out *dev, int64_t known_segments = -1,
                              const long long *known_kidx = nullptr, const uint64_t *known_len = nullptr);
int fd_posting_lengths_dev(fdgpu_ctx *c, const fdgpu_index *ix, const uint32_t *q_hash, uint64_t nq, uint64_t **dev_lengths);
uint64_t fd_maps_hashes(uint64_t n_queries, const fd_query_map *const *qms, std::vector<uint32_t> &h);
int fd_count_query_maps_len(fdgpu_ctx *c, const fdgpu_index *ix, uint64_t n_queries, const fd_query_map *const *qms, const uint64_t *len,
                            const uint64_t *primary_len, const float *penalty, float total_structures, uint32_t top_n, fd_count_rec **out,
                            uint64_t **out_off, fd_cq_dev_out *dev, const uint32_t *seg = nullptr, const long long *kidx = nullptr, bool allow_dense = true);
int fd_posting_lengths_segs(fdgpu_ctx *c, const fdgpu_index *ix, const uint32_t *q_hash, uint64_t nq, uint64_t *lengths, uint32_t *segs, long long *kidx = nullptr,
                            const uint8_t **land_out = nullptr);
int fd_count_query_maps_top_impl(fdgpu_ctx *c, const fdgpu_index *ix, uint64_t n_queries, const fd_query_map *const *qms, const float *penalty, float total_structures,
                                 uint32_t top_n, fd_count_rec **out, uint64_t **out_off, fd_cq_dev_out *dev, bool allow_dense = true);

struct fd_rb_dev_out { bool got = false; const void *recs = nullptr; const int32_t *residues = nullptr; uint64_t n_recs = 0, n_res = 0; };
int fd_retrieve_batch_dev(fdgpu_ctx *c, const fdgpu_batch *db, const uint8_t *resname_std, uint64_t n_queries, const uint32_t *cand, const uint64_t *cand_off,
                          const fd_query_map *const *qms, const fdgpu_batch *qb, const uint32_t *q_struct, const fd_hash_params *p, float ca_distance_cutoff,
                          uint32_t node_count, uint32_t partial_fit, fd_match_rec **matches, uint64_t **match_off, int32_t **residues, uint64_t **res_off, fd_rb_dev_out *dev);
hipError_t fd_d2h_to_file(fdgpu_ctx *c, int fd, uint64_t file_off, const void *src, size_t bytes, std::atomic<int> *io_err);
hipError_t fd_d2h_big(fdgpu_ctx *c, void *dst, const void *src, size_t bytes);
void *fd_out_alloc(size_t bytes, bool pinned = false);

void fd_launch_selfcheck(const fd_quant &q, uint32_t *out, hipStream_t st);
void fd_launch_hash_ok(const uint8_t *aa, const uint8_t *cb_valid, uint8_t *ok, uint64_t n, hipStream_t st);
void fd_launch_pair_count(const fd_batch_view &B, const fd_hash_consts &C, uint32_t *counts, hipStream_t st);
void fd_launch_pair_emit(const fd_batch_view &B, const fd_hash_consts &C, const uint64_t *seg_off, uint32_t *cursor, uint32_t *keys,
                         uint32_t *ids, uint32_t first_id, hipStream_t st);
void fd_launch_frames(const fd_batch_view &B, uint64_t n_res, void *frames, hipStream_t st);
void fd_launch_pair_count2(const fd_batch_view &B, const fd_hash_consts &C, uint32_t *counts, hipStream_t st);
void fd_launch_pair_emit2(const fd_batch_view &B, const void *frames, const fd_hash_consts &C, const uint64_t *seg_off, uint32_t *cursor,
                          uint32_t *keys, void *ids, bool ids16, uint32_t first_id, hipStream_t st);
int fd_radix_sort_pairs16(uint32_t *keys_a, uint16_t *vals_a, uint32_t *keys_b, uint16_t *vals_b, uint64_t n, int key_bits, uint32_t *ghist,
                          uint64_t *tot, hipStream_t st, fdgpu_ctx *timing_ctx = nullptr);
void fd_launch_frames_perm(const fd_batch_view &B, void *frames, float *ca_perm, uint8_t *ok_perm, uint8_t *aa_perm, unsigned long long *wide_flag, hipStream_t st);
void fd_launch_pair_count_msd(const fd_batch_view &B, const fd_hash_consts &C, uint32_t *counts, hipStream_t st);
void fd_launch_pair_emit_msd(const fd_batch_view &B, const void *frames, const fd_hash_consts &C, const uint64_t *seg_off, uint32_t *cursor, uint32_t *keys,
                             uint16_t *ids, hipStream_t st);
uint32_t fd_rs_seg_num_tiles(uint64_t n, uint32_t n_seg);
uint64_t fd_rs_seg_tot_words(uint64_t n, uint32_t n_seg);
size_t fd_rs_seg_tab_bytes(uint64_t n, uint32_t n_seg);
struct fd_rs_digit { uint32_t plane, shift; };
int fd_radix_sort_pairs16_seg(uint32_t *keys_a, uint16_t *vals_a, uint32_t *keys_b, uint16_t *vals_b, uint64_t n, const uint64_t *seg_off, uint64_t stride,
                              uint32_t n_seg, const fd_rs_digit *digits, int passes, uint32_t *ghist, uint64_t *tot, void *seg_tab, hipStream_t st, fdgpu_ctx *timing_ctx = nullptr,
                              unsigned long long *overflow = nullptr);
void fd_launch_row_count(const fd_batch_view &B, const fd_hash_consts &C, uint32_t *row_cnt, float cutoff, hipStream_t st);
void fd_launch_row_emit(const fd_batch_view &B, const fd_hash_consts &C, const uint64_t *row_off, uint32_t *keys, float cutoff, uint32_t *ids,
                        uint32_t first_id, hipStream_t st, int ids_partner = 0);
template <typename TIn>
void fd_exclusive_scan(const TIn *in, uint64_t n, uint64_t *out, uint64_t *chunk_tmp, uint64_t *total_dev, hipStream_t st);
uint64_t fd_scan_tmp_elems(uint64_t n);
uint32_t fd_rs_num_tiles(uint64_t n);
int fd_radix_sort_pairs(uint32_t *keys_a, uint32_t *vals_a, uint32_t *keys_b, uint32_t *vals_b, uint64_t n, int key_bits, uint32_t *ghist,
                        uint64_t *tot, hipStream_t st, fdgpu_ctx *timing_ctx = nullptr);
uint32_t fd_enc_num_tiles(uint64_t n);
void fd_launch_enc_sizes(const uint32_t *keys, const void *ids, int codec, uint32_t first_id, uint64_t n, uint32_t *tb, uint32_t *th, uint32_t *tp,
                         const uint64_t *seg_off, uint64_t S, uint64_t *bo, hipStream_t st);
void fd_launch_enc_write(const uint32_t *keys, const void *ids, int codec, uint32_t first_id, uint64_t n, const uint64_t *tbo, const uint64_t *tho,
                         uint8_t *value, uint32_t *hashes, uint64_t *offsets, uint32_t *last_ids, const uint64_t *total_bytes_dev, uint64_t H,
                         const uint64_t *bo, hipStream_t st);
void fd_launch_uniq_flags(const uint32_t *keys, const uint32_t *ids, uint64_t n, uint8_t *flags, hipStream_t st);
void fd_launch_compact(const uint32_t *keys, const uint8_t *flags, const uint64_t *pos, uint64_t n, uint32_t *out, hipStream_t st);
void fd_launch_gather_u64(const uint64_t *src, const uint64_t *idx, uint64_t n, uint64_t *dst, hipStream_t st);

struct cq_args {
    const uint32_t *hashes; const uint64_t *offsets; const uint8_t *value; uint64_t H;
    const uint32_t *q_hash; uint64_t nq;
    uint32_t *hash_bits;
    const unsigned long long *row_meta;
    uint32_t *match;
    unsigned long long *idf;
    int packed;
    uint32_t words; uint32_t first_id; uint32_t S;
};

#define QT_CELL_LOG2 11
#define QT_BINS 2048
#define QT_MAX_ROWS 1024
#define QT_MAXB 16
struct qt_state { uint32_t thr_bin, above, thr_key, count; };
struct qt_aux { uint32_t need_l2, shift2, edge, pad; };
struct qt_args {
    const uint8_t *value; const uint64_t *offsets;
    const unsigned long long *ck_meta; const uint2 *ck_ent;
    const long long *kidx;
    const unsigned long long *row_meta;
    const uint64_t *q_rows;
    const float *penalty;
    uint32_t nq, n_queries, S, first_id, NT, NC, tile_log2, plan_log2;
    uint4 *ranges;
    uint32_t *c_nid, *c_key;
    uint32_t *ccount;
    uint32_t *ghist;
    qt_state *state; qt_aux *aux;
    void *out; uint32_t cap;
    void *stream_ids; uint16_t *stream_row;
    uint2 *stream_tab;
    uint32_t *stream_used; uint32_t stream_cap;
    uint4 *pieces;
    uint32_t *piece_p;
    uint32_t *win;
    uint4 *heads;
    uint32_t win_per_row, top_n;
    uint32_t max_rows;
    const uint64_t *slices; uint32_t n_slices;
    unsigned long long *partial;
    uint32_t *g_bm, *g_rank, *g_tcount, *g_nid;
    uint32_t *g_rowbits; uint32_t g_wpr;
    const uint32_t *g_eend, *g_nend;
};
void fd_launch_ck_count(const uint64_t *offsets, uint64_t H, uint32_t NC, uint32_t *cnt, hipStream_t st);
void fd_launch_ck_fill(const uint64_t *offsets, const uint8_t *value, uint64_t H, uint32_t NC, uint32_t S, uint32_t first_id, const uint64_t *ent_off,
                       unsigned long long *meta, void *ent, hipStream_t st);
void fd_launch_qt_plan(const qt_args &A, hipStream_t st);
void fd_launch_qt_score(const qt_args &A, hipStream_t st);
void fd_launch_qt_big_score(const qt_args &A, hipStream_t st);
void fd_launch_qt_big_select(const qt_args &A, uint32_t top_n, void *sorted, hipStream_t st);
void fd_launch_qt_select(const qt_args &A, uint32_t top_n, void *sorted, hipStream_t st);
#define QT_WIN_CONT 0x80000000u
void fd_launch_qt_layout(const qt_args &A, hipStream_t st);
void fd_launch_qt_score32(const qt_args &A, hipStream_t st);

void fd_launch_index_lens(const uint64_t *offsets, const uint8_t *value, uint64_t H, uint32_t *lens, hipStream_t st);
void fd_launch_posting_lookup(const uint32_t *hashes, const uint64_t *offsets, const uint32_t *lens, uint64_t H, const uint32_t *q_hash, uint64_t nq, uint64_t *lengths,
                              uint32_t *nseg, long long *kidx, hipStream_t st);
void fd_launch_cq_plan(const cq_args &A, long long *kidx, uint32_t *nseg, hipStream_t st);
void fd_launch_cq_seg(const cq_args &A, const long long *kidx, const uint64_t *wstart, uint32_t *segsum, uint64_t n_items, bool split,
                      hipStream_t st);
void fd_launch_cq_rows_finalize(const cq_args &A, const uint64_t *q_rows, uint32_t n_queries, const uint64_t *slices, uint32_t n_slices, uint32_t *node_cnt,
                                uint32_t *edge_cnt, uint8_t *flags, uint64_t max_rows_per_query, hipStream_t st);

struct mp_query_dev {
    uint32_t qh_off, n_hashes;
    uint32_t aad_off, n_aad;
    uint32_t aa1_mask, aa2_mask;
    int use_prefilter;
    float ca_window;
    uint32_t qs_off, qs_mask;
};
#define MP_QH_LDS 1024
#define MP_SUBQ_STRIDE 16u
struct mp_args {
    fd_batch_view B;
    fd_hash_consts C;
    float cutoff;
    const uint32_t *cand; uint32_t n_cand;
    const uint32_t *wi_cand; const uint32_t *wi_i0; const uint32_t *wi_query; uint32_t n_work;
    const uint32_t *wi_j0; uint32_t j_span;
    const mp_query_dev *qtab;
    const uint32_t *qset;
    const uint8_t *resname_std;
    uint32_t aa1_mask, aa2_mask;
    int use_prefilter;
    const uint32_t *q_hashes; uint32_t n_hashes;
    const uint32_t *aad_start;
    const float *aad_dist; const uint32_t *aad_qi; uint32_t n_aad;
    const uint32_t *iv_start; const float2 *iv;
    const uint32_t *iv_grp;
    float ca_window;
    unsigned long long *n_found, *n_cands;
    const uint4 *cinfo; const uint32_t *act;
    unsigned long long *q_cnt; uint4 *chunk_hdr; uint32_t *chunk_ij; uint32_t cap_subq;
    uint32_t *res_h, *res_meta; float *res_d; uint2 *chunk_cnt; ulonglong2 *chunk_base;
    const uint32_t *bintab;
    int compact;
    fd_pair_rec *found; fd_cand_rec *cands;
    unsigned long long cap_found, cap_cands;
    uint32_t n_cfg;
    fd_quant qk[8];
    uint32_t mode;
    const uint32_t *cj_mask;
    const uint32_t *mask_off;
    uint32_t *votes; const uint64_t *vt_off; const uint32_t *vt_qs; const uint8_t *cj_comp;
    const float *sd_dist; const uint32_t *sd_qi;
};
struct fd_mp_tables {
    std::vector<uint32_t> blk; size_t o[13] = {0}; size_t nw = 0; bool want_iv = false; uint32_t j_span = 0; bool valid = false;
    const uint32_t *data = nullptr; size_t words = 0;
    bool dev_items = false; size_t o_wb = 0;
    uint64_t qset_slots = 0, qset_max_hashes = 0;
};
void fd_launch_mp_items(const uint32_t *db_res_off, const uint32_t *cand, uint32_t n_cand, const uint32_t *wbase, const uint32_t *cq, uint32_t j_span, uint32_t *wc,
                        uint32_t *wi, uint32_t *wq, uint32_t *wj, hipStream_t st, const uint8_t *aa, const uint8_t *hash_ok, const uint8_t *resname_std, int tert,
                        const struct mp_query_dev *qtab, void *cinfo , uint32_t *act );
struct fd_vote_plan {
    const uint8_t *cj_comp; uint64_t n_bits;
    const uint64_t *vt_off; const uint32_t *vt_qs; uint64_t n_counters;
    const uint64_t *row_off; const uint32_t *row_len; uint64_t n_rows;
    fd_vote_row *rows;
    const float *sd_dist; const uint32_t *sd_qi; uint64_t n_sd;
};
void fd_launch_vote_rows(const uint32_t *votes, const uint64_t *row_off, const uint32_t *row_len, uint64_t n_rows, fd_vote_row *out, hipStream_t st);
void fd_launch_match_pairs(const mp_args &A, hipStream_t st);
void fd_launch_mp_qset_build(const mp_query_dev *qtab, uint32_t n_queries, uint32_t max_hashes, const uint32_t *q_hashes, uint32_t *qset, hipStream_t st);
void fd_launch_found_key_ij(const fd_pair_rec *f, uint64_t n, uint32_t *key, uint32_t *val, hipStream_t st);
void fd_launch_found_key_slot(const fd_pair_rec *f, const uint32_t *val, uint64_t n, uint32_t *key, hipStream_t st);
void fd_launch_found_gather(const fd_pair_rec *f, const uint32_t *val, uint64_t n, fd_pair_rec *out, hipStream_t st);
void fd_launch_pack_cands(const fd_cand_rec *c, uint64_t n, uint32_t *key, uint32_t *val, hipStream_t st);
void fd_launch_kabsch(const float *x, const float *y, const uint64_t *off, uint64_t n, float *rmsd, float *rot, float *tran, hipStream_t st, uint64_t n_points = 0);
void fd_launch_metrics(const float *ref, const float *mov, const uint64_t *off, uint64_t n, const float *rot, const float *tran, const float *d0, float *out,
                       hipStream_t st, uint64_t n_points = 0);
void fd_launch_lms_qcp(const float *x, const float *y, const uint64_t *off, uint64_t n, float *rmsd, float *rot, float *tran, uint32_t *core_len,
                       uint8_t *flags, uint32_t *order, hipStream_t st);
void fd_launch_cq_compact_batch(const cq_args &A, const uint32_t *node_cnt, const uint32_t *edge_cnt, const uint8_t *flags, const uint64_t *pos,
                                const float *penalty, uint64_t total, void *out, hipStream_t st);
void fd_launch_cq_topn(const void *recs, const uint64_t *off, uint32_t n_queries, uint32_t top_n, uint32_t cap, void *out, void *state, uint32_t *ghist,
                       hipStream_t st);
void fd_launch_cq_topn_acc(const cq_args &A, const float *penalty, const uint32_t *node_cnt, const uint32_t *edge_cnt, uint32_t n_queries, uint32_t top_n,
                           uint32_t cap, void *out, void *state, uint32_t *ghist, hipStream_t st);
void fd_launch_cq_topn_dense(const cq_args &A, const uint64_t *q_rows, const float *penalty, uint32_t *keys, uint32_t n_queries, uint32_t top_n, uint32_t cap,
                             void *out, void *state, uint32_t *ghist, hipStream_t st);
void fd_launch_cq_topn_sort(const void *sel, uint32_t cap, const void *state, uint32_t n_queries, uint32_t top_n, void *out, hipStream_t st);
void fd_launch_get_entries(const uint32_t *hashes, const uint64_t *offsets, const uint8_t *value, uint64_t H, const uint32_t *q_hash, uint64_t nq,
                           const uint64_t *out_off, uint32_t *out, hipStream_t st);
struct rs_query_dev {
    uint32_t qh_off, n_hashes;
    uint32_t map_off;
    uint32_t idx_off, n_idx;
    uint32_t q_size;
    uint32_t q_res0;
    uint32_t pad;
};
struct rs_match_dev { uint32_t slot, ci, same, res_pos, prob0, prob1; float idf; uint32_t ord; };
#define RS_CNT_STRIDE 512
struct rs_args {
    const fd_pair_rec *found; const fd_cand_rec *cands;
    const uint32_t *seg_f, *seg_c, *perm_f, *perm_c;
    const uint32_t *cand, *slot_q;
    const uint32_t *order;
    uint32_t *slot_matches;
    const uint32_t *db_res_off; const float *db_ca, *db_cb, *q_ca, *q_cb;
    const rs_query_dev *qt;
    const uint32_t *hashes, *kfirst; const uint8_t *sym;
    const uint32_t *map_qi, *map_qj; const float *map_idf;
    const uint32_t *indices;
    const float *d0tab;
    uint32_t node_count;
    uint32_t node_cap;
    unsigned long long *counters;
    uint32_t *flags;
    rs_match_dev *matches; int32_t *residues; float *kx, *ky; uint64_t *koff; float *d0;
    uint32_t *gq, *gr;
    uint64_t cap_matches, cap_res, cap_prob, cap_pts;
    uint4 *sp_edges;
    uint32_t *sp_nodes;
    unsigned long long *sp_comps;
    uint4 *sp_head;
    uint2 *sp_work;
    uint4 *sp_np;
    uint32_t *sp_gq, *sp_gr;
    uint32_t *sp_big, *sp_big_n;
    const uint32_t *n_listed;
};
void fd_launch_rs_group(const fd_pair_rec *found, uint64_t nf, const fd_cand_rec *cands, uint64_t nc, uint32_t n_cand, uint32_t *cnt, uint32_t *seg, uint32_t *cur,
                        uint32_t *perm_f, uint32_t *perm_c, hipStream_t st);
void fd_launch_rs_slots(const rs_args &A, uint32_t n_cand, hipStream_t st);
void fd_launch_rs_points(const rs_args &A, uint64_t n_prob, uint64_t n_points, hipStream_t st);
void fd_launch_rs_records_dev(const void *matches, uint64_t n, const uint32_t *slot_matches, uint32_t n_cand, const uint64_t *cand_off, const uint32_t *slot_q,
                              const rs_query_dev *qt, uint32_t n_queries, uint32_t *scratch, uint64_t *match_off, uint64_t *res_off, const float *rmsd,
                              const float *rot, const float *tran, const float *met, const int32_t *residues, void *out, int32_t *out_res, hipStream_t st);
int fd_match_pairs_multi(fdgpu_ctx *c, const fdgpu_batch *db, const uint8_t *resname_std, uint64_t n_queries, const fd_match_query *qs,
                         const uint32_t *cand, const uint64_t *cand_off, const fd_hash_params *p, fd_pair_rec **found, uint64_t *n_found,
                         fd_cand_rec **cands, uint64_t *n_cands, uint32_t mode = 3, const uint32_t *cj_mask = nullptr,
                         const uint32_t *mask_off = nullptr, uint64_t mask_words = 0, uint32_t **pk_key = nullptr, uint32_t **pk_val = nullptr,
                         fd_vote_plan *votes = nullptr, struct fd_mp_tables *tables = nullptr, const std::function<void()> *while_scanning = nullptr);
```

### folddisco_amd/csrc/k_hash.hip

```cpp
#include "fd_device.h"
#include "fd_geom_other.h"
#ifndef FD_EMIT_WAVES
#define FD_EMIT_WAVES 5
#endif
#define FD_MSD_BUCKETS 40u

__global__ __launch_bounds__(FD_WAVE) void k_pair_count(fd_batch_view B, fd_hash_consts C, uint32_t *__restrict__ counts) {
    uint32_t w = fd_xcd_remap(blockIdx.x, B.n_work);
    if (w >= B.n_work) return;
    const uint32_t s = B.wi_struct[w];
    const uint32_t r0 = B.res_off[s], r1 = B.res_off[s + 1];
    const uint32_t i = B.wi_i0[w] + threadIdx.x;
    const bool vi = i < r1 && B.hash_ok[i];
    fd_v3 cai = {0.f, 0.f, 0.f};
    if (vi) cai = fd_load3(B.ca_xyz, i);
    uint32_t cnt = 0;
    for (uint32_t j = r0; j < r1; ++j) {
        if (!B.hash_ok[j]) continue;
        fd_v3 caj = fd_load3(B.ca_xyz, j);
        float d2 = fd_dist2(cai, caj);
        cnt += (vi && i != j && !(d2 > C.d2_max)) ? 1u : 0u;
    }
    for (int off = 32; off > 0; off >>= 1) cnt += __shfl_down(cnt, off, FD_WAVE);
    if (threadIdx.x == 0 && cnt) atomicAdd(&counts[s], cnt);
}

template <bool WRITE_IDS>
__device__ __forceinline__ void drain(const fd_batch_view &B, const fd_hash_consts &C, const uint32_t *q, uint32_t n,
                                      uint32_t i0, uint32_t r0, uint32_t s, uint32_t id, const uint64_t *seg_off,
                                      uint32_t *cursor, uint32_t *keys, uint32_t *ids) {
    const uint32_t lane = threadIdx.x;
    uint32_t base = 0;
    if (lane == 0) base = atomicAdd(&cursor[s], n);
    base = __shfl(base, 0, FD_WAVE);
    if (lane < n) {
        uint32_t e = q[lane];
        uint32_t i = i0 + (e >> 16), j = r0 + (e & 0xffffu);
        fd_v3 n1 = fd_load3(B.n_xyz, i), ca1 = fd_load3(B.ca_xyz, i), cb1 = fd_load3(B.cb_xyz, i);
        fd_v3 n2 = fd_load3(B.n_xyz, j), ca2 = fd_load3(B.ca_xyz, j), cb2 = fd_load3(B.cb_xyz, j);
        fd_feature f = fd_pair_feature(n1, ca1, cb1, n2, ca2, cb2);
        uint32_t h = fd_hash_enc(B.aa[i], B.aa[j], f, C.q);
        uint64_t pos = seg_off[s] + base + lane;
        keys[pos] = h;
        if (WRITE_IDS) ids[pos] = id;
    }
}

template <bool WRITE_IDS>
__global__ __launch_bounds__(FD_WAVE) void k_pair_emit(fd_batch_view B, fd_hash_consts C, const uint64_t *__restrict__ seg_off,
                                                       uint32_t *__restrict__ cursor, uint32_t *__restrict__ keys,
                                                       uint32_t *__restrict__ ids, uint32_t first_id) {
    __shared__ uint32_t q[2 * FD_WAVE];
    uint32_t w = fd_xcd_remap(blockIdx.x, B.n_work);
    if (w >= B.n_work) return;
    const uint32_t s = B.wi_struct[w];
    const uint32_t r0 = B.res_off[s], r1 = B.res_off[s + 1];
    const uint32_t i0 = B.wi_i0[w];
    const uint32_t lane = threadIdx.x;
    const uint32_t i = i0 + lane;
    const bool vi = i < r1 && B.hash_ok[i];
    fd_v3 cai = {0.f, 0.f, 0.f};
    if (vi) cai = fd_load3(B.ca_xyz, i);
    uint32_t qn = 0;
    for (uint32_t j = r0; j < r1; ++j) {
        if (!B.hash_ok[j]) continue;
        fd_v3 caj = fd_load3(B.ca_xyz, j);
        float d2 = fd_dist2(cai, caj);
        bool pass = vi && i != j && !(d2 > C.d2_max);
        uint64_t m = __ballot(pass);
        if (m == 0) continue;
        if (pass) q[qn + fd_mbcnt(m)] = (lane << 16) | (j - r0);
        qn += (uint32_t)__popcll(m);
        if (qn >= FD_WAVE) {
            __syncthreads();
            qn -= FD_WAVE;
            drain<WRITE_IDS>(B, C, q + qn, FD_WAVE, i0, r0, s, first_id + s, seg_off, cursor, keys, ids);
            __syncthreads();
        }
    }
    if (qn) {
        __syncthreads();
        drain<WRITE_IDS>(B, C, q, qn, i0, r0, s, first_id + s, seg_off, cursor, keys, ids);
    }
}

__global__ __launch_bounds__(256) void k_frames(fd_batch_view B, uint32_t n_res, fd_frame *__restrict__ frames) {
    uint32_t r = blockIdx.x * blockDim.x + threadIdx.x;
    if (r >= n_res) return;
    fd_frame F;
    if (B.hash_ok[r]) F = fd_make_frame(fd_load3(B.n_xyz, r), fd_load3(B.ca_xyz, r), fd_load3(B.cb_xyz, r));
    else { F = fd_frame{}; F.ca = fd_load3(B.ca_xyz, r); }
    F.pad = __uint_as_float((uint32_t)B.aa[r]);
    frames[r] = F;
}

typedef float fd_f2 __attribute__((ext_vector_type(2)));
#define FD_NOT_HASHABLE 0x100u

__device__ __forceinline__ bool fd_lane_of(uint64_t m) { return __builtin_amdgcn_inverse_ballot_w64(m); }

template <bool TYPES, class Step, class RunEnd>
__device__ __forceinline__ void fd_filter_block(const fd_batch_view &B, float d2_max, const fd_v3 &cai, uint64_t vim, uint32_t i0, uint32_t jb, uint32_t r1,
                                                float *s_cj, Step &&step, RunEnd &&run_end) {
    const uint32_t lane = threadIdx.x;
    const uint32_t jl = jb + lane;
    fd_v3 cj = {0.f, 0.f, 0.f};
    uint32_t kind = FD_NOT_HASHABLE;
    if (jl < r1) {
        cj = fd_load3(B.ca_xyz, jl);
        if (B.hash_ok[jl]) kind = TYPES ? (uint32_t)B.aa[jl] : 0u;
    }
    fd_wave_lds_fence();
    s_cj[lane] = cj.x; s_cj[FD_WAVE + lane] = cj.y; s_cj[2 * FD_WAVE + lane] = cj.z;
    fd_wave_lds_fence();
    const uint64_t okm = __ballot(kind != FD_NOT_HASHABLE);
    const uint64_t starts = __ballot(kind != (uint32_t)__shfl_up((int)kind, 1, FD_WAVE)) | 1ull;
    const bool last_block = jb + FD_WAVE >= r1;
    const uint32_t nk = okm ? 64u - (uint32_t)__builtin_clzll(okm) : 0u;
    const uint32_t nkf = (last_block && nk == 0) ? 1u : nk;
    const bool first = jb == i0;
    const fd_f2 ax = {cai.x, cai.x}, ay = {cai.y, cai.y}, az = {cai.z, cai.z};
    uint32_t k = 0;
    while (k < nkf) {
        const uint32_t t = (uint32_t)__builtin_amdgcn_readlane((int)kind, (int)k);
        const uint64_t rest = (starts >> k) >> 1;
        uint32_t ke = rest ? k + 1u + (uint32_t)__builtin_ctzll(rest) : (uint32_t)FD_WAVE;
        ke = ke < nkf ? ke : nkf;
        const bool run_last = last_block && ke >= nkf;
        const bool dead = t == FD_NOT_HASHABLE;
        if (dead && !run_last) { k = ke; continue; }
        const uint64_t vr = dead ? 0ull : vim;
        uint64_t gt = first ? (1ull << k) - 1ull : ~0ull;
        do {
            const fd_f2 xj = {s_cj[k], s_cj[k + 1]}, yj = {s_cj[FD_WAVE + k], s_cj[FD_WAVE + k + 1]}, zj = {s_cj[2 * FD_WAVE + k], s_cj[2 * FD_WAVE + k + 1]};
            const fd_f2 dx = ax - xj, dy = ay - yj, dz = az - zj;
            const fd_f2 d2 = (dx * dx + dy * dy) + dz * dz;
            const uint64_t gt1 = gt << 1 | 1ull;
            const uint64_t m0 = __ballot(!(d2.x > d2_max)) & vr & gt;
            const uint64_t m1 = (k + 1u < ke) ? (__ballot(!(d2.y > d2_max)) & vr & gt1) : 0ull;
            gt = gt1 << 1 | 1ull;
            const uint32_t k0 = k;
            k += 2;
            step(k0, t, m0, m1, run_last && k >= ke);
        } while (k < ke);
        k = ke;
        run_end(t);
    }
}

__global__ __launch_bounds__(FD_WAVE) void k_pair_count2(fd_batch_view B, fd_hash_consts C, uint32_t *__restrict__ counts) {
    __shared__ float s_cj[3 * FD_WAVE + 1];
    uint32_t w = fd_xcd_remap(blockIdx.x, B.n_work);
    if (w >= B.n_work) return;
    const uint32_t s = B.wi_struct[w];
    const uint32_t r1 = B.res_off[s + 1];
    const uint32_t i0 = B.wi_i0[w];
    const uint32_t i = i0 + threadIdx.x;
    const bool vi = i < r1 && B.hash_ok[i];
    fd_v3 cai = {0.f, 0.f, 0.f};
    if (vi) cai = fd_load3(B.ca_xyz, i);
    const uint64_t vim = __ballot(vi);
    uint32_t cnt = 0;
    for (uint32_t jb = i0; jb < r1; jb += FD_WAVE)
        fd_filter_block<false>(B, C.d2_max, cai, vim, i0, jb, r1, s_cj,
                               [&](uint32_t, uint32_t, uint64_t m0, uint64_t m1, bool) { cnt += (fd_lane_of(m0) ? 1u : 0u) + (fd_lane_of(m1) ? 1u : 0u); },
                               [](uint32_t) {});
    cnt *= 2u;
    for (int off = 32; off > 0; off >>= 1) cnt += __shfl_down(cnt, off, FD_WAVE);
    if (threadIdx.x == 0 && cnt) atomicAdd(&counts[s], cnt);
}

__global__ __launch_bounds__(256) void k_frames_perm(fd_batch_view B, fd_frame *__restrict__ frames, float *__restrict__ ca_perm, uint8_t *__restrict__ ok_perm,
                                                     uint8_t *__restrict__ aa_perm, unsigned long long *__restrict__ wide_flag) {
    __shared__ uint32_t cnt[32], cur[32];
    const uint32_t s = blockIdx.x;
    const uint32_t r0 = B.res_off[s], r1 = B.res_off[s + 1];
    if (threadIdx.x < 32) cnt[threadIdx.x] = 0;
    __syncthreads();
    for (uint32_t r = r0 + threadIdx.x; r < r1; r += 256) {
        const uint32_t a = B.aa[r];
        atomicAdd(&cnt[(B.hash_ok[r] && a < 20u) ? a : 20u], 1u);
    }
    __syncthreads();
    if (threadIdx.x == 0) { uint32_t run = 0; for (int k = 0; k < 21; ++k) { cur[k] = run; run += cnt[k]; } }
    __syncthreads();
    for (uint32_t r = r0 + threadIdx.x; r < r1; r += 256) {
        const uint32_t a = B.aa[r];
        bool ok = B.hash_ok[r] != 0;
        if (ok && a >= 20u) {
            ok = false;
            if (wide_flag) atomicOr(wide_flag, 1ull);
        }
        const uint32_t p = r0 + atomicAdd(&cur[(ok && a < 20u) ? a : 20u], 1u);
        fd_frame F;
        const fd_v3 ca = fd_load3(B.ca_xyz, r);
        if (ok) F = fd_make_frame(fd_load3(B.n_xyz, r), ca, fd_load3(B.cb_xyz, r));
        else { F = fd_frame{}; F.ca = ca; }
        F.pad = __uint_as_float(a);
        frames[p] = F;
        ca_perm[3ull * p] = ca.x; ca_perm[3ull * p + 1] = ca.y; ca_perm[3ull * p + 2] = ca.z;
        ok_perm[p] = ok ? 1 : 0;
        aa_perm[p] = (uint8_t)a;
    }
}

__global__ __launch_bounds__(FD_WAVE) void k_pair_count_msd(fd_batch_view B, fd_hash_consts C, uint32_t *__restrict__ counts) {
    __shared__ uint32_t s_cnt[FD_WAVE];
    __shared__ float s_cj[3 * FD_WAVE + 1];
    uint32_t w = fd_xcd_remap(blockIdx.x, B.n_work);
    if (w >= B.n_work) return;
    const uint32_t s = B.wi_struct[w];
    const uint32_t r1 = B.res_off[s + 1];
    const uint32_t i0 = B.wi_i0[w];
    const uint32_t lane = threadIdx.x;
    const uint32_t i = i0 + lane;
    const bool vi = i < r1 && B.hash_ok[i];
    fd_v3 cai = {0.f, 0.f, 0.f};
    uint32_t aai = 0;
    if (vi) { cai = fd_load3(B.ca_xyz, i); aai = B.aa[i]; }
    s_cnt[lane] = 0;
    __syncthreads();
    const uint64_t vim = __ballot(vi);
    uint32_t c_lo = 0, c_hi = 0, run = 0;
    const uint32_t hi_i = aai >> 4;
    for (uint32_t jb = i0; jb < r1; jb += FD_WAVE)
        fd_filter_block<true>(B, C.d2_max, cai, vim, i0, jb, r1, s_cj,
                              [&](uint32_t, uint32_t, uint64_t m0, uint64_t m1, bool) { run += (fd_lane_of(m0) ? 1u : 0u) + (fd_lane_of(m1) ? 1u : 0u); },
                              [&](uint32_t t) {
                                  if (t >= 16u) c_hi += run; else c_lo += run;
                                  if (run) atomicAdd(&s_cnt[(t * 2u + hi_i) & (FD_WAVE - 1u)], run);
                                  run = 0;
                              });
    if (c_lo) atomicAdd(&s_cnt[aai * 2u], c_lo);
    if (c_hi) atomicAdd(&s_cnt[aai * 2u + 1u], c_hi);
    __syncthreads();
    if (lane < FD_MSD_BUCKETS && s_cnt[lane]) atomicAdd(&counts[(uint64_t)lane * B.n_struct + s], s_cnt[lane]);
}

__device__ __forceinline__ fd_frame load_frame(const fd_frame *__restrict__ frames, uint32_t r) {
    const float4 *p = reinterpret_cast<const float4 *>(frames + r);
    float4 a = p[0], b = p[1], c = p[2], d = p[3], e = p[4];
    fd_frame F;
    F.ca = {a.x, a.y, a.z}; F.cb = {a.w, b.x, b.y}; F.r1 = {b.z, b.w, c.x}; F.t1 = {c.y, c.z, c.w};
    F.len = d.x; F.pad = d.y; F.s2 = {d.z, d.w, e.x}; F.nv2 = {e.y, e.z, e.w};
    return F;
}
__device__ __forceinline__ fd_frame hot_frame(const float4 &a, const float4 &b, const float4 &c, const float4 &d) {
    fd_frame F{};
    F.ca = {a.x, a.y, a.z}; F.cb = {a.w, b.x, b.y}; F.r1 = {b.z, b.w, c.x}; F.t1 = {c.y, c.z, c.w};
    F.len = d.x; F.pad = d.y;
    return F;
}

__device__ __attribute__((noinline)) uint2 pair_both_tab_exact(const fd_frame *__restrict__ frames, uint32_t i, uint32_t j, uint32_t aai,
                                                               uint32_t aaj, float dist_disc, float ang_disc, const uint32_t *tab) {
    fd_frame Fi = load_frame(frames, i), Fj = load_frame(frames, j);
    fd_quant q;
    q.dist_disc = dist_disc; q.ang_disc = ang_disc; q.ang2_disc = 0.0f; q.type = FD_HASH_PDBTR;
    uint32_t a, b;
    fd_pair_both_tab(Fi, Fj, aai, aaj, q, tab, &a, &b);
    return make_uint2(a, b);
}

template <int TAB, bool IDS16, bool MSD, bool DT = false>
__device__ __forceinline__ void drain2(const fd_batch_view &B, const fd_frame *__restrict__ frames, const fd_hash_consts &C,
                                       const uint32_t *tab, const uint32_t *q, uint32_t n, uint32_t i0, uint32_t r0, uint32_t s, uint32_t id,
                                       const uint64_t *seg_off, uint32_t *cursor, uint32_t *keys, void *ids, const float4 *s_fi,
                                       uint32_t *s_bc, uint64_t *s_bb, const uint64_t *s_boff) {
    const uint32_t lane = threadIdx.x;
    uint32_t base = 0, gb = 0, slots = 0;
    if (!MSD) {
        if (lane == 0) base = atomicAdd(&cursor[s], 2u * n);
        base = __shfl(base, 0, FD_WAVE);
    } else {
        s_bc[lane] = 0;
        fd_wave_lds_fence();
        if (lane < n) {
            const uint32_t e = q[lane], il = (e >> 16) & 63u, aj = e >> 22;
            const uint32_t ai = TAB == 2 ? __float_as_uint(s_fi[192 + il].y) : (uint32_t)B.aa[i0 + il];
            const uint32_t bf = ai * 2u + (aj >> 4), br = aj * 2u + (ai >> 4);
            slots = atomicAdd(&s_bc[bf], 1u) | atomicAdd(&s_bc[br], 1u) << 8 | bf << 16 | br << 24;
        }
        fd_wave_lds_fence();
        if (lane < FD_MSD_BUCKETS) { const uint32_t c = s_bc[lane]; if (c) gb = atomicAdd(&cursor[(uint64_t)lane * B.n_struct + s], c); }
    }
    uint32_t h_ij = 0, h_ji = 0, aai = 0, aaj = 0;
    if (lane < n) {
        uint32_t e = q[lane];
        uint32_t i = i0 + ((e >> 16) & 63u), j = r0 + (e & 0xffffu);
        if (TAB == 2) {
            const uint32_t il = (e >> 16) & 63u;
            const fd_frame Fi = hot_frame(s_fi[il], s_fi[64 + il], s_fi[128 + il], s_fi[192 + il]);
            const float4 *pj = reinterpret_cast<const float4 *>(frames + j);
            const fd_frame Fj = hot_frame(pj[0], pj[1], pj[2], pj[3]);
            aai = __float_as_uint(Fi.pad); aaj = __float_as_uint(Fj.pad);
#if defined(FD_EMIT_STUB) && FD_EMIT_STUB == 1
            h_ij = aai << 25 | aaj << 20 | (__float_as_uint(Fj.ca.x) & 0xfffffu); h_ji = aaj << 25 | aai << 20 | (__float_as_uint(Fi.ca.x) & 0xfffffu);
            if (false)
#endif
            if (!fd_pair_both_spec<DT>(Fi, Fj, aai, aaj, C.q, tab, tab + 32, &h_ij, &h_ji, tab + 64)) {
                uint2 h = pair_both_tab_exact(frames, i, j, B.aa[i], B.aa[j], C.q.dist_disc, C.q.ang_disc, tab);
                h_ij = h.x; h_ji = h.y;
                if (C.spec_miss) atomicAdd(C.spec_miss, 1ull);
            }
        } else if (TAB == 1) {
            uint2 h = pair_both_tab_exact(frames, i, j, B.aa[i], B.aa[j], C.q.dist_disc, C.q.ang_disc, tab);
            h_ij = h.x; h_ji = h.y;
        } else {
            fd_frame Fi = load_frame(frames, i), Fj = load_frame(frames, j);
            fd_pair_both(Fi, Fj, B.aa[i], B.aa[j], C.q, &h_ij, &h_ji);
        }
    }
    if (MSD) {
        asm volatile("" : "+v"(gb));
        if (lane < FD_MSD_BUCKETS) s_bb[lane] = s_boff[lane] + gb;
        fd_wave_lds_fence();
        if (lane < n) {
            const uint32_t sf = slots & 255u, sr = (slots >> 8) & 255u, bf = (slots >> 16) & 255u, br = slots >> 24;
            if ((((h_ij | h_ji) >> 30) || (h_ij >> 24) != bf || (h_ji >> 24) != br) && C.wide_flag) atomicOr(C.wide_flag, 1ull);
            const uint64_t pf = s_bb[bf] + sf, pr = s_bb[br] + sr;
            keys[pf] = (h_ij << 24) | s;
            keys[pr] = (h_ji << 24) | s;
            ((uint16_t *)ids)[pf] = (uint16_t)(h_ij >> 8);
            ((uint16_t *)ids)[pr] = (uint16_t)(h_ji >> 8);
        }
        return;
    }
    if (lane < n) {
        const uint64_t so = seg_off[s];
        uint64_t pos = so * C.seg_mul + (uint64_t)C.seg_cfg * (seg_off[s + 1] - so) + base + lane;
        if (IDS16) {
            if (((h_ij | h_ji) >> 30) && C.wide_flag) atomicOr(C.wide_flag, 1ull);
            uint32_t hi = s >> 16;
            uint16_t lo = (uint16_t)(s & 0xffffu);
            keys[pos] = (h_ij << 2) | hi;
            keys[pos + n] = (h_ji << 2) | hi;
            ((uint16_t *)ids)[pos] = lo;
            ((uint16_t *)ids)[pos + n] = lo;
        } else {
            keys[pos] = h_ij;
            keys[pos + n] = h_ji;
            ((uint32_t *)ids)[pos] = id;
            ((uint32_t *)ids)[pos + n] = id;
        }
    }
}

template <int TAB, bool IDS16, bool MSD, bool DT = false>
__global__ __launch_bounds__(FD_WAVE, FD_EMIT_WAVES) void k_pair_emit2(fd_batch_view B, const fd_frame *__restrict__ frames, fd_hash_consts C,
                                                        const uint64_t *__restrict__ seg_off, uint32_t *__restrict__ cursor,
                                                        uint32_t *__restrict__ keys, void *__restrict__ ids, uint32_t first_id) {
    __shared__ uint32_t q[3 * FD_WAVE];
    __shared__ float s_cj[3 * FD_WAVE + 1];
    __shared__ uint32_t tab[DT ? 64 + FD_DIST_NTHR + 1 : 64];
    uint32_t w = fd_xcd_remap(blockIdx.x, B.n_work);
    if (w >= B.n_work) return;
    if (TAB) {
        if (DT && threadIdx.x < FD_DIST_NTHR) tab[64 + threadIdx.x] = fd_dist_thr_bits[threadIdx.x];
        if (threadIdx.x == 0) {
            fd_fill_bintab(tab);
            for (int k = 0; k < FD_BINTAB_WORDS; ++k) tab[32 + k] = tab[k];
            for (int m = 0; m < 4; ++m)
                for (int k = 0; k < 4; ++k) { uint32_t v = tab[32 + 7 + 5 * m + k]; tab[32 + 7 + 5 * m + k] = v > 0x7f7fffffu ? 0x7f7fffffu : v; }
        }
        __syncthreads();
    }
    const uint32_t s = B.wi_struct[w];
    const uint32_t r0 = B.res_off[s], r1 = B.res_off[s + 1];
    const uint32_t i0 = B.wi_i0[w];
    const uint32_t lane = threadIdx.x;
    const uint32_t i = i0 + lane;
    const bool vi = i < r1 && B.hash_ok[i];
    fd_v3 cai = {0.f, 0.f, 0.f};
    if (vi) cai = fd_load3(B.ca_xyz, i);
    __shared__ float4 s_fi[4 * FD_WAVE];
    if (TAB == 2 && i < r1) {
        const float4 *fp = reinterpret_cast<const float4 *>(frames + i);
#pragma unroll
        for (int k = 0; k < 4; ++k) s_fi[k * FD_WAVE + lane] = fp[k];
    }
    __shared__ uint32_t s_bc[MSD ? FD_WAVE : 1];
    __shared__ uint64_t s_bb[MSD ? FD_MSD_BUCKETS : 1], s_boff[MSD ? FD_MSD_BUCKETS : 1];
    if (MSD && lane < FD_MSD_BUCKETS) s_boff[lane] = seg_off[(uint64_t)lane * B.n_struct + s];
    __syncthreads();
    const uint64_t vim = __ballot(vi);
    const uint32_t lane16 = lane << 16;
    uint32_t qn = 0;
    for (uint32_t jb = i0; jb < r1; jb += FD_WAVE) {
        const uint32_t jrel = jb - r0;
        fd_filter_block<MSD>(B, C.d2_max, cai, vim, i0, jb, r1, s_cj,
            [&](uint32_t k, uint32_t t, uint64_t m0, uint64_t m1, bool last) {
                const uint32_t tag = (MSD ? t << 22 : 0u) | (jrel + k);
                if (m0) {
                    if (fd_lane_of(m0)) q[__builtin_amdgcn_mbcnt_hi((uint32_t)(m0 >> 32), __builtin_amdgcn_mbcnt_lo((uint32_t)m0, qn))] = lane16 | tag;
                    qn += (uint32_t)__popcll(m0);
                }
                if (m1) {
                    if (fd_lane_of(m1)) q[__builtin_amdgcn_mbcnt_hi((uint32_t)(m1 >> 32), __builtin_amdgcn_mbcnt_lo((uint32_t)m1, qn))] = lane16 | (tag + 1u);
                    qn += (uint32_t)__popcll(m1);
                }
                while (qn >= FD_WAVE || (last && qn)) {
                    fd_wave_lds_fence();
                    uint32_t n = qn < FD_WAVE ? qn : FD_WAVE;
                    qn -= n;
                    drain2<TAB, IDS16, MSD, DT>(B, frames, C, tab, q + qn, n, i0, r0, s, first_id + s, seg_off, cursor, keys, ids, s_fi, s_bc, s_bb, s_boff);
                    fd_wave_lds_fence();
                }
            },
            [](uint32_t) {});
    }
}

__global__ __launch_bounds__(FD_WAVE) void k_row_count(fd_batch_view B, fd_hash_consts C, uint32_t *__restrict__ row_cnt, float cutoff) {
    uint32_t w = fd_xcd_remap(blockIdx.x, B.n_work);
    if (w >= B.n_work) return;
    const uint32_t s = B.wi_struct[w];
    const uint32_t r0 = B.res_off[s], r1 = B.res_off[s + 1];
    const uint32_t i = B.wi_i0[w] + threadIdx.x;
    if (i >= r1) return;
    if (fd_own_descriptor(C.q.type)) {
        uint32_t cnt = 0;
        if (B.aa[i] != 255)
            for (uint32_t j = r0; j < r1; ++j)
                cnt += (j != i && B.aa[j] != 255 && fd_accept_other(C.q.type, B, r0, r1, i, j, cutoff)) ? 1u : 0u;
        row_cnt[i] = cnt;
        return;
    }
    const bool vi = B.hash_ok[i];
    fd_v3 cai = fd_load3(B.ca_xyz, i);
    uint32_t cnt = 0;
    for (uint32_t j = r0; j < r1; ++j) {
        if (!B.hash_ok[j]) continue;
        float d2 = fd_dist2(cai, fd_load3(B.ca_xyz, j));
        cnt += (vi && i != j && !(d2 > C.d2_max)) ? 1u : 0u;
    }
    row_cnt[i] = cnt;
}

__global__ __launch_bounds__(FD_WAVE) void k_row_emit(fd_batch_view B, fd_hash_consts C, const uint64_t *__restrict__ row_off,
                                                      uint32_t *__restrict__ keys, float cutoff, uint32_t *__restrict__ ids, uint32_t first_id, int ids_partner) {
    uint32_t w = fd_xcd_remap(blockIdx.x, B.n_work);
    if (w >= B.n_work) return;
    const uint32_t s = B.wi_struct[w];
    const uint32_t r0 = B.res_off[s], r1 = B.res_off[s + 1];
    const uint32_t i = B.wi_i0[w] + threadIdx.x;
    if (i >= r1) return;
    if (fd_own_descriptor(C.q.type)) {
        if (B.aa[i] == 255) return;
        uint64_t pos = row_off[i];
        float f[FD_NFEAT];
        for (uint32_t j = r0; j < r1; ++j) {
            if (j == i || B.aa[j] == 255 || !fd_feature_other(C.q.type, B, r0, r1, i, j, cutoff, f)) continue;
            if (ids) ids[pos] = ids_partner ? j : first_id + s;
            keys[pos++] = fd_hash_other(C.q.type, f, C.q);
        }
        return;
    }
    if (!B.hash_ok[i]) return;
    fd_v3 n1 = fd_load3(B.n_xyz, i), ca1 = fd_load3(B.ca_xyz, i), cb1 = fd_load3(B.cb_xyz, i);
    uint32_t aa1 = B.aa[i];
    uint64_t pos = row_off[i];
    for (uint32_t j = r0; j < r1; ++j) {
        if (!B.hash_ok[j] || i == j) continue;
        fd_v3 ca2 = fd_load3(B.ca_xyz, j);
        if (fd_dist2(ca1, ca2) > C.d2_max) continue;
        fd_v3 n2 = fd_load3(B.n_xyz, j), cb2 = fd_load3(B.cb_xyz, j);
        fd_feature f = fd_pair_feature(n1, ca1, cb1, n2, ca2, cb2);
        if (ids) ids[pos] = ids_partner ? j : first_id + s;
        keys[pos++] = fd_hash_enc(aa1, B.aa[j], f, C.q);
    }
}

__global__ void k_hash_ok(const uint8_t *__restrict__ aa, const uint8_t *__restrict__ cb_valid, uint8_t *__restrict__ ok, uint64_t n) {
    uint64_t k = (uint64_t)blockIdx.x * blockDim.x + threadIdx.x;
    if (k < n) ok[k] = (aa[k] != 255 && (cb_valid == nullptr || cb_valid[k])) ? 1 : 0;
}

__global__ void k_selfcheck(fd_quant q, uint32_t *__restrict__ out ) {
    if (threadIdx.x != 0 || blockIdx.x != 0) return;
    const fd_v3 N[3] = {{6.661f, 8.291f, 43.860f}, {10.483f, 7.756f, 49.260f}, {5.260f, -1.068f, 41.296f}};
    const fd_v3 CA[3] = {{6.994f, 8.354f, 42.405f}, {9.429f, 7.479f, 48.266f}, {5.547f, 0.158f, 42.050f}};
    const fd_v3 CB[3] = {{8.251f, 7.488f, 42.026f}, {10.033f, 6.489f, 47.255f}, {5.773f, 1.360f, 41.130f}};
    const uint32_t AA[3] = {8u, 3u, 15u};
    const int PI[6] = {1, 1, 0, 0, 2, 2}, PJ[6] = {0, 2, 1, 2, 1, 0};
    uint32_t tab[64 + FD_DIST_NTHR + 1];
    fd_fill_bintab(tab);
    for (int k = 0; k < FD_BINTAB_WORDS; ++k) tab[32 + k] = tab[k];
    for (int m = 0; m < 4; ++m)
        for (int k = 0; k < 4; ++k) { uint32_t v = tab[32 + 7 + 5 * m + k]; tab[32 + 7 + 5 * m + k] = v > 0x7f7fffffu ? 0x7f7fffffu : v; }
    for (int k = 0; k < FD_DIST_NTHR; ++k) tab[64 + k] = fd_dist_thr_bits[k];
    fd_frame F[3];
    for (int r = 0; r < 3; ++r) F[r] = fd_make_frame(N[r], CA[r], CB[r]);
    for (int k = 0; k < 6; ++k) {
        const int i = PI[k], j = PJ[k];
        out[k] = fd_hash_pdbtr(AA[i], AA[j], fd_pair_feature(N[i], CA[i], CB[i], N[j], CA[j], CB[j]), q);
        uint32_t a, b;
        fd_pair_both_tab(F[i], F[j], AA[i], AA[j], q, tab, &a, &b);
        out[6 + k] = a;
        if (!fd_pair_both_spec(F[i], F[j], AA[i], AA[j], q, tab, tab + 32, &a, &b)) fd_pair_both_tab(F[i], F[j], AA[i], AA[j], q, tab, &a, &b);
        out[12 + k] = a;
        if (!fd_pair_both_spec<true>(F[i], F[j], AA[i], AA[j], q, tab, tab + 32, &a, &b, tab + 64)) fd_pair_both_tab(F[i], F[j], AA[i], AA[j], q, tab, &a, &b);
        out[18 + k] = a;
    }
}

extern "C++" {
void fd_launch_selfcheck(const fd_quant &q, uint32_t *out, hipStream_t st) { hipLaunchKernelGGL(k_selfcheck, dim3(1), dim3(64), 0, st, q, out); }
void fd_launch_hash_ok(const uint8_t *aa, const uint8_t *cb_valid, uint8_t *ok, uint64_t n, hipStream_t st) {
    if (!n) return;
    hipLaunchKernelGGL(k_hash_ok, dim3((unsigned)((n + 255) / 256)), dim3(256), 0, st, aa, cb_valid, ok, n);
}
static inline unsigned grid_for(uint32_t n_work) { return ((n_work + 7u) / 8u) * 8u; }
void fd_launch_pair_count(const fd_batch_view &B, const fd_hash_consts &C, uint32_t *counts, hipStream_t st) {
    if (!B.n_work) return;
    hipLaunchKernelGGL(k_pair_count, dim3(grid_for(B.n_work)), dim3(FD_WAVE), 0, st, B, C, counts);
}
void fd_launch_pair_emit(const fd_batch_view &B, const fd_hash_consts &C, const uint64_t *seg_off, uint32_t *cursor,
                         uint32_t *keys, uint32_t *ids, uint32_t first_id, hipStream_t st) {
    if (!B.n_work) return;
    if (ids)
        hipLaunchKernelGGL(k_pair_emit<true>, dim3(grid_for(B.n_work)), dim3(FD_WAVE), 0, st, B, C, seg_off, cursor, keys, ids, first_id);
    else
        hipLaunchKernelGGL(k_pair_emit<false>, dim3(grid_for(B.n_work)), dim3(FD_WAVE), 0, st, B, C, seg_off, cursor, keys, ids, first_id);
}
void fd_launch_frames(const fd_batch_view &B, uint64_t n_res, void *frames, hipStream_t st) {
    if (!n_res) return;
    hipLaunchKernelGGL(k_frames, dim3((unsigned)((n_res + 255) / 256)), dim3(256), 0, st, B, (uint32_t)n_res, (fd_frame *)frames);
}
void fd_launch_pair_count2(const fd_batch_view &B, const fd_hash_consts &C, uint32_t *counts, hipStream_t st) {
    if (!B.n_work) return;
    hipLaunchKernelGGL(k_pair_count2, dim3(grid_for(B.n_work)), dim3(FD_WAVE), 0, st, B, C, counts);
}
void fd_launch_pair_emit2(const fd_batch_view &B, const void *frames, const fd_hash_consts &C, const uint64_t *seg_off, uint32_t *cursor,
                          uint32_t *keys, void *ids, bool ids16, uint32_t first_id, hipStream_t st) {
    if (!B.n_work) return;
    dim3 g(grid_for(B.n_work)), b(FD_WAVE);
    const fd_frame *F = (const fd_frame *)frames;
    if (C.use_tab >= 2 && ids16) hipLaunchKernelGGL((k_pair_emit2<2, true, false>), g, b, 0, st, B, F, C, seg_off, cursor, keys, ids, first_id);
    else if (C.use_tab >= 2) hipLaunchKernelGGL((k_pair_emit2<2, false, false>), g, b, 0, st, B, F, C, seg_off, cursor, keys, ids, first_id);
    else if (C.use_tab && ids16) hipLaunchKernelGGL((k_pair_emit2<1, true, false>), g, b, 0, st, B, F, C, seg_off, cursor, keys, ids, first_id);
    else if (C.use_tab) hipLaunchKernelGGL((k_pair_emit2<1, false, false>), g, b, 0, st, B, F, C, seg_off, cursor, keys, ids, first_id);
    else if (ids16) hipLaunchKernelGGL((k_pair_emit2<0, true, false>), g, b, 0, st, B, F, C, seg_off, cursor, keys, ids, first_id);
    else hipLaunchKernelGGL((k_pair_emit2<0, false, false>), g, b, 0, st, B, F, C, seg_off, cursor, keys, ids, first_id);
}
void fd_launch_frames_perm(const fd_batch_view &B, void *frames, float *ca_perm, uint8_t *ok_perm, uint8_t *aa_perm, unsigned long long *wide_flag, hipStream_t st) {
    if (!B.n_struct) return;
    hipLaunchKernelGGL(k_frames_perm, dim3(B.n_struct), dim3(256), 0, st, B, (fd_frame *)frames, ca_perm, ok_perm, aa_perm, wide_flag);
}
void fd_launch_pair_count_msd(const fd_batch_view &B, const fd_hash_consts &C, uint32_t *counts, hipStream_t st) {
    if (!B.n_work) return;
    hipLaunchKernelGGL(k_pair_count_msd, dim3(grid_for(B.n_work)), dim3(FD_WAVE), 0, st, B, C, counts);
}
void fd_launch_pair_emit_msd(const fd_batch_view &B, const void *frames, const fd_hash_consts &C, const uint64_t *seg_off, uint32_t *cursor, uint32_t *keys,
                             uint16_t *ids, hipStream_t st) {
    if (!B.n_work) return;
    dim3 g(grid_for(B.n_work)), b(FD_WAVE);
    const fd_frame *F = (const fd_frame *)frames;
    if (C.use_tab == 3) hipLaunchKernelGGL((k_pair_emit2<2, true, true, true>), g, b, 0, st, B, F, C, seg_off, cursor, keys, (void *)ids, 0u);
    else if (C.use_tab == 2) hipLaunchKernelGGL((k_pair_emit2<2, true, true>), g, b, 0, st, B, F, C, seg_off, cursor, keys, (void *)ids, 0u);
    else if (C.use_tab) hipLaunchKernelGGL((k_pair_emit2<1, true, true>), g, b, 0, st, B, F, C, seg_off, cursor, keys, (void *)ids, 0u);
    else hipLaunchKernelGGL((k_pair_emit2<0, true, true>), g, b, 0, st, B, F, C, seg_off, cursor, keys, (void *)ids, 0u);
}
void fd_launch_row_count(const fd_batch_view &B, const fd_hash_consts &C, uint32_t *row_cnt, float cutoff, hipStream_t st) {
    if (!B.n_work) return;
    hipLaunchKernelGGL(k_row_count, dim3(grid_for(B.n_work)), dim3(FD_WAVE), 0, st, B, C, row_cnt, cutoff);
}
void fd_launch_row_emit(const fd_batch_view &B, const fd_hash_consts &C, const uint64_t *row_off, uint32_t *keys, float cutoff, uint32_t *ids,
                        uint32_t first_id, hipStream_t st, int ids_partner) {
    if (!B.n_work) return;
    hipLaunchKernelGGL(k_row_emit, dim3(grid_for(B.n_work)), dim3(FD_WAVE), 0, st, B, C, row_off, keys, cutoff, ids, first_id, ids_partner);
}
}
```

Before: 1.590 million structures/s.

## Key MSD segments per work item and fold frame build into pair count

New measurement: 1.647 million structures/s, median of 6. 1.04x the previous value.

```diff
diff --git a/folddisco_amd/csrc/fdgpu_api.hip b/folddisco_amd/csrc/fdgpu_api.hip
--- a/folddisco_amd/csrc/fdgpu_api.hip
+++ b/folddisco_amd/csrc/fdgpu_api.hip
@@ -631,7 +631,7 @@
 extern "C" uint64_t fdgpu_index_num_structures(const fdgpu_index *ix) { return ix ? ix->n_structures : 0; }
 
 #define FDGPU_RETRY_WIDE 1000
-static int encode_sorted_stream(fdgpu_ctx *c, const uint32_t *ks, const void *is, int codec, uint64_t first_id, uint64_t P, uint64_t S, fdgpu_index **out) {
+static int encode_sorted_stream(fdgpu_ctx *c, const uint32_t *ks, const void *is, int codec, uint64_t first_id, uint64_t P, uint64_t S, uint64_t seg_stride, fdgpu_index **out) {
     hipStream_t st = c->stream;
     const bool el6 = codec != 0;
     int rc;
@@ -651,7 +651,7 @@
         HIPCHK(c, hipMemsetAsync(c->ws[WS_TILE_H].p, 0, (size_t)(nt + 1) * 4, st));
         HIPCHK(c, hipMemsetAsync(c->ws[WS_TILE_P].p, 0, (size_t)(nt + 1) * 4, st));
         fd_launch_enc_sizes(ks, is, codec, (uint32_t)first_id, P, c->ws[WS_TILE_B].as<uint32_t>(), c->ws[WS_TILE_H].as<uint32_t>(), c->ws[WS_TILE_P].as<uint32_t>(),
-                            c->ws[WS_SEGOFF].as<uint64_t>(), S, c->ws[WS_MISC3].as<uint64_t>() + 8, st);
+                            c->ws[WS_SEGOFF].as<uint64_t>(), seg_stride, c->ws[WS_MISC3].as<uint64_t>() + 8, st);
         uint64_t *totd = c->ws[WS_MISC3].as<uint64_t>();
         fd_exclusive_scan<uint32_t>(c->ws[WS_TILE_B].as<uint32_t>(), nt_eff, c->ws[WS_TILE_BO].as<uint64_t>(), c->ws[WS_SCANTMP].as<uint64_t>(), totd + 0, st);
         fd_exclusive_scan<uint32_t>(c->ws[WS_TILE_H].as<uint32_t>(), nt_eff, c->ws[WS_TILE_HO].as<uint64_t>(), c->ws[WS_SCANTMP].as<uint64_t>(), totd + 1, st);
@@ -705,8 +705,10 @@
         HIPCHK(c, c->ws[WS_CA_PERM].ensure(std::max<uint64_t>(b->n_res, 1) * 12));
         HIPCHK(c, c->ws[WS_OK_PERM].ensure(std::max<uint64_t>(b->n_res, 1)));
         HIPCHK(c, c->ws[WS_AA_PERM].ensure(std::max<uint64_t>(b->n_res, 1)));
-        StageTimer t(c, "frames", b->n_res * (37 + sizeof(fd_frame) + 14));
-        fd_launch_frames_perm(V, c->ws[WS_FRAMES].p, c->ws[WS_CA_PERM].as<float>(), c->ws[WS_OK_PERM].as<uint8_t>(), c->ws[WS_AA_PERM].as<uint8_t>(), C.wide_flag, st);
+        HIPCHK(c, c->ws[WS_SRC_PERM].ensure(std::max<uint64_t>(b->n_res, 1) * 4));
+        StageTimer t(c, "frames", b->n_res * (2 + 14 + 18));
+        fd_launch_frames_perm(V, c->ws[WS_CA_PERM].as<float>(), c->ws[WS_OK_PERM].as<uint8_t>(), c->ws[WS_AA_PERM].as<uint8_t>(), c->ws[WS_SRC_PERM].as<uint32_t>(),
+                              C.wide_flag, st);
         V.ca_xyz = c->ws[WS_CA_PERM].as<float>(); V.hash_ok = c->ws[WS_OK_PERM].as<uint8_t>(); V.aa = c->ws[WS_AA_PERM].as<uint8_t>();
         V.n_xyz = nullptr; V.cb_xyz = nullptr;
     } else {
@@ -731,17 +733,14 @@
         HIPCHK(c, hipGetLastError());
         rc = d2h_u64(c, c->ws[WS_TOTAL].as<uint64_t>(), &P1);
     } else if (msd) {
-        const uint64_t NS = NB * S;
+        const uint64_t NS = NB * b->n_work;
         HIPCHK(c, c->ws[WS_COUNTS].ensure((NS + 1) * 4));
-        HIPCHK(c, c->ws[WS_CURSOR].ensure((NS + 1) * 4));
         HIPCHK(c, c->ws[WS_SEGOFF].ensure((NS + 2) * 8));
         HIPCHK(c, c->ws[WS_SCANTMP].ensure(fd_scan_tmp_elems(std::max<uint64_t>(NS, b->n_res)) * 8 + 64));
         HIPCHK(c, c->ws[WS_TOTAL].ensure(64));
-        HIPCHK(c, hipMemsetAsync(c->ws[WS_COUNTS].p, 0, (NS + 1) * 4, st));
-        HIPCHK(c, hipMemsetAsync(c->ws[WS_CURSOR].p, 0, (NS + 1) * 4, st));
         {
-            StageTimer t(c, "pair_count", b->n_res * 14);
-            fd_launch_pair_count_msd(V, C, c->ws[WS_COUNTS].as<uint32_t>(), st);
+            StageTimer t(c, "pair_count", b->n_res * (14 + 28 + sizeof(fd_frame)) + NS * 4);
+            fd_launch_pair_count_msd(V, C, b->n_xyz, b->cb_xyz, c->ws[WS_SRC_PERM].as<uint32_t>(), c->ws[WS_FRAMES].p, c->ws[WS_COUNTS].as<uint32_t>(), st);
         }
         {
             StageTimer t(c, "segment_scan", NS * 12);
@@ -766,7 +765,7 @@
     {
         StageTimer t(c, "pair_emit", b->n_res * 37 + P * (el6 ? 6 : 8));
         if (own) fd_launch_row_emit(b->view(), C, c->ws[WS_MISC1].as<uint64_t>(), ka, p->dist_cutoff, (uint32_t *)ia, (uint32_t)first_id, st);
-        else if (msd) fd_launch_pair_emit_msd(V, c->ws[WS_FRAMES].p, C, c->ws[WS_SEGOFF].as<uint64_t>(), c->ws[WS_CURSOR].as<uint32_t>(), ka, (uint16_t *)ia, st);
+        else if (msd) fd_launch_pair_emit_msd(V, c->ws[WS_FRAMES].p, C, c->ws[WS_SEGOFF].as<uint64_t>(), ka, (uint16_t *)ia, st);
         else for (uint32_t k = 0; k < n_cfg; ++k) {
             fd_hash_consts Ck = fd_make_consts_cfg(p, k);
             Ck.spec_miss = C.spec_miss; Ck.wide_flag = C.wide_flag; Ck.seg_mul = n_cfg; Ck.seg_cfg = k;
@@ -781,13 +780,13 @@
         HIPCHK(c, c->ws[WS_GHIST].ensure((size_t)256 * fd_rs_seg_num_tiles(P, NB) * 4));
         HIPCHK(c, c->ws[WS_TOT].ensure(fd_rs_seg_tot_words(P, NB) * 8));
         HIPCHK(c, c->ws[WS_SEG_TAB].ensure(fd_rs_seg_tab_bytes(P, NB)));
-        cur = fd_radix_sort_pairs16_seg(ka, (uint16_t *)ia, kb, (uint16_t *)ib, P, c->ws[WS_SEGOFF].as<uint64_t>(), S, NB, digits, 3, c->ws[WS_GHIST].as<uint32_t>(),
+        cur = fd_radix_sort_pairs16_seg(ka, (uint16_t *)ia, kb, (uint16_t *)ib, P, c->ws[WS_SEGOFF].as<uint64_t>(), b->n_work, NB, digits, 3, c->ws[WS_GHIST].as<uint32_t>(),
                                         c->ws[WS_TOT].as<uint64_t>(), c->ws[WS_SEG_TAB].p, st, c, c->ws[WS_MISC3].as<unsigned long long>() + 4);
     } else if (ids16) cur = fd_radix_sort_pairs16(ka, (uint16_t *)ia, kb, (uint16_t *)ib, P, 32, c->ws[WS_GHIST].as<uint32_t>(), c->ws[WS_TOT].as<uint64_t>(), st, c);
     else cur = sort_pairs(c, ka, (uint32_t *)ia, kb, (uint32_t *)ib, P, 32);
     const uint32_t *ks = cur ? kb : ka;
     const void *is = cur ? ib : ia;
-    return encode_sorted_stream(c, ks, is, codec, first_id, P, S, out);
+    return encode_sorted_stream(c, ks, is, codec, first_id, P, S, msd ? b->n_work : 0, out);
 }
 
 extern "C" int fdgpu_index_build(fdgpu_ctx *c, const fdgpu_batch *b, const fd_hash_params *p, uint64_t first_id, fdgpu_index **out) { FD_LOCK(c);
@@ -816,7 +815,7 @@
         HIPCHK(c, hipMemcpyAsync(c->ws[WS_KEYS_A].p, hashes, n * 4, hipMemcpyHostToDevice, st));
         HIPCHK(c, hipMemcpyAsync(c->ws[WS_IDS_A].p, ids, n * 4, hipMemcpyHostToDevice, st));
     }
-    return encode_sorted_stream(c, c->ws[WS_KEYS_A].as<uint32_t>(), c->ws[WS_IDS_A].p, 0, 0, n, S, out);
+    return encode_sorted_stream(c, c->ws[WS_KEYS_A].as<uint32_t>(), c->ws[WS_IDS_A].p, 0, 0, n, S, 0, out);
 }
 
 #define FD_PIN_SLOTS 16
diff --git a/folddisco_amd/csrc/fdgpu_internal.h b/folddisco_amd/csrc/fdgpu_internal.h
--- a/folddisco_amd/csrc/fdgpu_internal.h
+++ b/folddisco_amd/csrc/fdgpu_internal.h
@@ -87,7 +87,7 @@
     WS_TILE_B, WS_TILE_H, WS_TILE_P, WS_TILE_BO, WS_TILE_HO , WS_TILE_PO, WS_MISC0, WS_MISC1, WS_MISC2, WS_MISC3, WS_MISC4, WS_MISC5, WS_FRAMES,
     WS_CQ_KIDX, WS_CQ_NSEG, WS_CQ_WSTART, WS_CQ_SEGSUM, WS_CQ_TOPN,
     WS_QT_RANGES, WS_QT_COMPACT, WS_QT_COUNT, WS_QT_AUX, WS_RS_PLAN, WS_RS_REC, WS_RS_RECRES, WS_QT_PARTIAL, WS_QT_SURV, WS_QT_ROWBITS, WS_QT_STREAM, WS_QT_STAB, WS_QT_PIECEP, WS_QT_WIN, WS_QT_HEAD, WS_RS_SPLIT, WS_MP_QSET,
-    WS_CA_PERM, WS_OK_PERM, WS_AA_PERM, WS_SEG_TAB,
+    WS_CA_PERM, WS_OK_PERM, WS_AA_PERM, WS_SRC_PERM , WS_SEG_TAB,
     WS_RS_TAB, WS_RS_SEG, WS_RS_OUT, WS_RS_RES, WS_RS_KX, WS_RS_KY, WS_RS_KOFF, WS_RS_SOL, WS_RS_CNT, WS_RS_GQ, WS_MP_ACT, WS_MP_Q,
     WS_SG_TAB , WS_SG_TAB_B, WS_SG_PAIRS, WS_SG_CURSOR,
     WS_SG_NB_PART , WS_SG_NB_OUT ,
@@ -289,9 +289,10 @@
                           uint32_t *keys, void *ids, bool ids16, uint32_t first_id, hipStream_t st);
 int fd_radix_sort_pairs16(uint32_t *keys_a, uint16_t *vals_a, uint32_t *keys_b, uint16_t *vals_b, uint64_t n, int key_bits, uint32_t *ghist,
                           uint64_t *tot, hipStream_t st, fdgpu_ctx *timing_ctx = nullptr);
-void fd_launch_frames_perm(const fd_batch_view &B, void *frames, float *ca_perm, uint8_t *ok_perm, uint8_t *aa_perm, unsigned long long *wide_flag, hipStream_t st);
-void fd_launch_pair_count_msd(const fd_batch_view &B, const fd_hash_consts &C, uint32_t *counts, hipStream_t st);
-void fd_launch_pair_emit_msd(const fd_batch_view &B, const void *frames, const fd_hash_consts &C, const uint64_t *seg_off, uint32_t *cursor, uint32_t *keys,
+void fd_launch_frames_perm(const fd_batch_view &B, float *ca_perm, uint8_t *ok_perm, uint8_t *aa_perm, uint32_t *src_perm, unsigned long long *wide_flag, hipStream_t st);
+void fd_launch_pair_count_msd(const fd_batch_view &B, const fd_hash_consts &C, const float *n_xyz, const float *cb_xyz, const uint32_t *src_perm, void *frames,
+                              uint32_t *counts, hipStream_t st);
+void fd_launch_pair_emit_msd(const fd_batch_view &B, const void *frames, const fd_hash_consts &C, const uint64_t *seg_off, uint32_t *keys,
                              uint16_t *ids, hipStream_t st);
 uint32_t fd_rs_seg_num_tiles(uint64_t n, uint32_t n_seg);
 uint64_t fd_rs_seg_tot_words(uint64_t n, uint32_t n_seg);
diff --git a/folddisco_amd/csrc/k_hash.hip b/folddisco_amd/csrc/k_hash.hip
--- a/folddisco_amd/csrc/k_hash.hip
+++ b/folddisco_amd/csrc/k_hash.hip
@@ -170,10 +170,10 @@
     if (threadIdx.x == 0 && cnt) atomicAdd(&counts[s], cnt);
 }
 
-__global__ __launch_bounds__(256) void k_frames_perm(fd_batch_view B, fd_frame *__restrict__ frames, float *__restrict__ ca_perm, uint8_t *__restrict__ ok_perm,
-                                                     uint8_t *__restrict__ aa_perm, unsigned long long *__restrict__ wide_flag) {
-    __shared__ uint32_t cnt[32], cur[32];
-    const uint32_t s = blockIdx.x;
+__global__ __launch_bounds__(256) void k_frames_perm(fd_batch_view B, float *__restrict__ ca_perm, uint8_t *__restrict__ ok_perm, uint8_t *__restrict__ aa_perm,
+                                                     uint32_t *__restrict__ src_perm, unsigned long long *__restrict__ wide_flag) {
+    __shared__ uint32_t cnt[32], cur[32], wcnt[4][32];
+    const uint32_t s = blockIdx.x, lane = threadIdx.x & (FD_WAVE - 1u), wave = threadIdx.x / FD_WAVE;
     const uint32_t r0 = B.res_off[s], r1 = B.res_off[s + 1];
     if (threadIdx.x < 32) cnt[threadIdx.x] = 0;
     __syncthreads();
@@ -184,27 +184,46 @@
     __syncthreads();
     if (threadIdx.x == 0) { uint32_t run = 0; for (int k = 0; k < 21; ++k) { cur[k] = run; run += cnt[k]; } }
     __syncthreads();
-    for (uint32_t r = r0 + threadIdx.x; r < r1; r += 256) {
-        const uint32_t a = B.aa[r];
-        bool ok = B.hash_ok[r] != 0;
-        if (ok && a >= 20u) {
-            ok = false;
-            if (wide_flag) atomicOr(wide_flag, 1ull);
-        }
-        const uint32_t p = r0 + atomicAdd(&cur[(ok && a < 20u) ? a : 20u], 1u);
-        fd_frame F;
-        const fd_v3 ca = fd_load3(B.ca_xyz, r);
-        if (ok) F = fd_make_frame(fd_load3(B.n_xyz, r), ca, fd_load3(B.cb_xyz, r));
-        else { F = fd_frame{}; F.ca = ca; }
-        F.pad = __uint_as_float(a);
-        frames[p] = F;
-        ca_perm[3ull * p] = ca.x; ca_perm[3ull * p + 1] = ca.y; ca_perm[3ull * p + 2] = ca.z;
-        ok_perm[p] = ok ? 1 : 0;
-        aa_perm[p] = (uint8_t)a;
-    }
-}
-
-__global__ __launch_bounds__(FD_WAVE) void k_pair_count_msd(fd_batch_view B, fd_hash_consts C, uint32_t *__restrict__ counts) {
+    for (uint32_t rb = r0; rb < r1; rb += 256) {
+        const uint32_t r = rb + threadIdx.x;
+        uint32_t a = 0, cls = 21u;
+        bool ok = false;
+        if (r < r1) {
+            a = B.aa[r];
+            ok = B.hash_ok[r] != 0;
+            if (ok && a >= 20u) {
+                ok = false;
+                if (wide_flag) atomicOr(wide_flag, 1ull);
+            }
+            cls = ok ? a : 20u;
+        }
+        uint64_t mine = 0;
+        uint32_t wc = 0;
+#pragma unroll 1
+        for (uint32_t k = 0; k < 21u; ++k) {
+            const uint64_t m = __ballot(cls == k);
+            if (cls == k) mine = m;
+            if (lane == k) wc = (uint32_t)__popcll(m);
+        }
+        if (lane < 21u) wcnt[wave][lane] = wc;
+        __syncthreads();
+        if (r < r1) {
+            uint32_t p = r0 + cur[cls] + fd_mbcnt(mine);
+            for (uint32_t v = 0; v < wave; ++v) p += wcnt[v][cls];
+            const fd_v3 ca = fd_load3(B.ca_xyz, r);
+            ca_perm[3ull * p] = ca.x; ca_perm[3ull * p + 1] = ca.y; ca_perm[3ull * p + 2] = ca.z;
+            ok_perm[p] = ok ? 1 : 0;
+            aa_perm[p] = (uint8_t)a;
+            src_perm[p] = r;
+        }
+        __syncthreads();
+        if (threadIdx.x < 21u) cur[threadIdx.x] += wcnt[0][threadIdx.x] + wcnt[1][threadIdx.x] + wcnt[2][threadIdx.x] + wcnt[3][threadIdx.x];
+        __syncthreads();
+    }
+}
+
+__global__ __launch_bounds__(FD_WAVE) void k_pair_count_msd(fd_batch_view B, fd_hash_consts C, const float *__restrict__ n_xyz, const float *__restrict__ cb_xyz,
+                                                            const uint32_t *__restrict__ src_perm, fd_frame *__restrict__ frames, uint32_t *__restrict__ counts) {
     __shared__ uint32_t s_cnt[FD_WAVE];
     __shared__ float s_cj[3 * FD_WAVE + 1];
     uint32_t w = fd_xcd_remap(blockIdx.x, B.n_work);
@@ -218,6 +237,13 @@
     fd_v3 cai = {0.f, 0.f, 0.f};
     uint32_t aai = 0;
     if (vi) { cai = fd_load3(B.ca_xyz, i); aai = B.aa[i]; }
+    if (i < r1) {
+        fd_frame F;
+        if (vi) { const uint32_t src = src_perm[i]; F = fd_make_frame(fd_load3(n_xyz, src), cai, fd_load3(cb_xyz, src)); }
+        else { F = fd_frame{}; F.ca = fd_load3(B.ca_xyz, i); }
+        F.pad = __uint_as_float((uint32_t)B.aa[i]);
+        frames[i] = F;
+    }
     s_cnt[lane] = 0;
     __syncthreads();
     const uint64_t vim = __ballot(vi);
@@ -234,7 +260,7 @@
     if (c_lo) atomicAdd(&s_cnt[aai * 2u], c_lo);
     if (c_hi) atomicAdd(&s_cnt[aai * 2u + 1u], c_hi);
     __syncthreads();
-    if (lane < FD_MSD_BUCKETS && s_cnt[lane]) atomicAdd(&counts[(uint64_t)lane * B.n_struct + s], s_cnt[lane]);
+    if (lane < FD_MSD_BUCKETS) counts[(uint64_t)lane * B.n_work + w] = s_cnt[lane];
 }
 
 __device__ __forceinline__ fd_frame load_frame(const fd_frame *__restrict__ frames, uint32_t r) {
@@ -266,9 +292,9 @@
 __device__ __forceinline__ void drain2(const fd_batch_view &B, const fd_frame *__restrict__ frames, const fd_hash_consts &C,
                                        const uint32_t *tab, const uint32_t *q, uint32_t n, uint32_t i0, uint32_t r0, uint32_t s, uint32_t id,
                                        const uint64_t *seg_off, uint32_t *cursor, uint32_t *keys, void *ids, const float4 *s_fi,
-                                       uint32_t *s_bc, uint64_t *s_bb, const uint64_t *s_boff) {
+                                       uint32_t *s_bc, uint64_t *s_boff) {
     const uint32_t lane = threadIdx.x;
-    uint32_t base = 0, gb = 0, slots = 0;
+    uint32_t base = 0, slots = 0;
     if (!MSD) {
         if (lane == 0) base = atomicAdd(&cursor[s], 2u * n);
         base = __shfl(base, 0, FD_WAVE);
@@ -281,8 +307,6 @@
             const uint32_t bf = ai * 2u + (aj >> 4), br = aj * 2u + (ai >> 4);
             slots = atomicAdd(&s_bc[bf], 1u) | atomicAdd(&s_bc[br], 1u) << 8 | bf << 16 | br << 24;
         }
-        fd_wave_lds_fence();
-        if (lane < FD_MSD_BUCKETS) { const uint32_t c = s_bc[lane]; if (c) gb = atomicAdd(&cursor[(uint64_t)lane * B.n_struct + s], c); }
     }
     uint32_t h_ij = 0, h_ji = 0, aai = 0, aaj = 0;
     if (lane < n) {
@@ -312,18 +336,17 @@
         }
     }
     if (MSD) {
-        asm volatile("" : "+v"(gb));
-        if (lane < FD_MSD_BUCKETS) s_bb[lane] = s_boff[lane] + gb;
-        fd_wave_lds_fence();
         if (lane < n) {
             const uint32_t sf = slots & 255u, sr = (slots >> 8) & 255u, bf = (slots >> 16) & 255u, br = slots >> 24;
             if ((((h_ij | h_ji) >> 30) || (h_ij >> 24) != bf || (h_ji >> 24) != br) && C.wide_flag) atomicOr(C.wide_flag, 1ull);
-            const uint64_t pf = s_bb[bf] + sf, pr = s_bb[br] + sr;
+            const uint64_t pf = s_boff[bf] + sf, pr = s_boff[br] + sr;
             keys[pf] = (h_ij << 24) | s;
             keys[pr] = (h_ji << 24) | s;
             ((uint16_t *)ids)[pf] = (uint16_t)(h_ij >> 8);
             ((uint16_t *)ids)[pr] = (uint16_t)(h_ji >> 8);
         }
+        fd_wave_lds_fence();
+        if (lane < FD_MSD_BUCKETS) s_boff[lane] += s_bc[lane];
         return;
     }
     if (lane < n) {
@@ -380,8 +403,8 @@
         for (int k = 0; k < 4; ++k) s_fi[k * FD_WAVE + lane] = fp[k];
     }
     __shared__ uint32_t s_bc[MSD ? FD_WAVE : 1];
-    __shared__ uint64_t s_bb[MSD ? FD_MSD_BUCKETS : 1], s_boff[MSD ? FD_MSD_BUCKETS : 1];
-    if (MSD && lane < FD_MSD_BUCKETS) s_boff[lane] = seg_off[(uint64_t)lane * B.n_struct + s];
+    __shared__ uint64_t s_boff[MSD ? FD_MSD_BUCKETS : 1];
+    if (MSD && lane < FD_MSD_BUCKETS) s_boff[lane] = seg_off[(uint64_t)lane * B.n_work + w];
     __syncthreads();
     const uint64_t vim = __ballot(vi);
     const uint32_t lane16 = lane << 16;
@@ -403,7 +426,7 @@
                     fd_wave_lds_fence();
                     uint32_t n = qn < FD_WAVE ? qn : FD_WAVE;
                     qn -= n;
-                    drain2<TAB, IDS16, MSD, DT>(B, frames, C, tab, q + qn, n, i0, r0, s, first_id + s, seg_off, cursor, keys, ids, s_fi, s_bc, s_bb, s_boff);
+                    drain2<TAB, IDS16, MSD, DT>(B, frames, C, tab, q + qn, n, i0, r0, s, first_id + s, seg_off, cursor, keys, ids, s_fi, s_bc, s_boff);
                     fd_wave_lds_fence();
                 }
             },
@@ -543,23 +566,24 @@
     else if (ids16) hipLaunchKernelGGL((k_pair_emit2<0, true, false>), g, b, 0, st, B, F, C, seg_off, cursor, keys, ids, first_id);
     else hipLaunchKernelGGL((k_pair_emit2<0, false, false>), g, b, 0, st, B, F, C, seg_off, cursor, keys, ids, first_id);
 }
-void fd_launch_frames_perm(const fd_batch_view &B, void *frames, float *ca_perm, uint8_t *ok_perm, uint8_t *aa_perm, unsigned long long *wide_flag, hipStream_t st) {
+void fd_launch_frames_perm(const fd_batch_view &B, float *ca_perm, uint8_t *ok_perm, uint8_t *aa_perm, uint32_t *src_perm, unsigned long long *wide_flag, hipStream_t st) {
     if (!B.n_struct) return;
-    hipLaunchKernelGGL(k_frames_perm, dim3(B.n_struct), dim3(256), 0, st, B, (fd_frame *)frames, ca_perm, ok_perm, aa_perm, wide_flag);
-}
-void fd_launch_pair_count_msd(const fd_batch_view &B, const fd_hash_consts &C, uint32_t *counts, hipStream_t st) {
-    if (!B.n_work) return;
-    hipLaunchKernelGGL(k_pair_count_msd, dim3(grid_for(B.n_work)), dim3(FD_WAVE), 0, st, B, C, counts);
-}
-void fd_launch_pair_emit_msd(const fd_batch_view &B, const void *frames, const fd_hash_consts &C, const uint64_t *seg_off, uint32_t *cursor, uint32_t *keys,
+    hipLaunchKernelGGL(k_frames_perm, dim3(B.n_struct), dim3(256), 0, st, B, ca_perm, ok_perm, aa_perm, src_perm, wide_flag);
+}
+void fd_launch_pair_count_msd(const fd_batch_view &B, const fd_hash_consts &C, const float *n_xyz, const float *cb_xyz, const uint32_t *src_perm, void *frames,
+                              uint32_t *counts, hipStream_t st) {
+    if (!B.n_work) return;
+    hipLaunchKernelGGL(k_pair_count_msd, dim3(grid_for(B.n_work)), dim3(FD_WAVE), 0, st, B, C, n_xyz, cb_xyz, src_perm, (fd_frame *)frames, counts);
+}
+void fd_launch_pair_emit_msd(const fd_batch_view &B, const void *frames, const fd_hash_consts &C, const uint64_t *seg_off, uint32_t *keys,
                              uint16_t *ids, hipStream_t st) {
     if (!B.n_work) return;
     dim3 g(grid_for(B.n_work)), b(FD_WAVE);
     const fd_frame *F = (const fd_frame *)frames;
-    if (C.use_tab == 3) hipLaunchKernelGGL((k_pair_emit2<2, true, true, true>), g, b, 0, st, B, F, C, seg_off, cursor, keys, (void *)ids, 0u);
-    else if (C.use_tab == 2) hipLaunchKernelGGL((k_pair_emit2<2, true, true>), g, b, 0, st, B, F, C, seg_off, cursor, keys, (void *)ids, 0u);
-    else if (C.use_tab) hipLaunchKernelGGL((k_pair_emit2<1, true, true>), g, b, 0, st, B, F, C, seg_off, cursor, keys, (void *)ids, 0u);
-    else hipLaunchKernelGGL((k_pair_emit2<0, true, true>), g, b, 0, st, B, F, C, seg_off, cursor, keys, (void *)ids, 0u);
+    if (C.use_tab == 3) hipLaunchKernelGGL((k_pair_emit2<2, true, true, true>), g, b, 0, st, B, F, C, seg_off, (uint32_t *)nullptr, keys, (void *)ids, 0u);
+    else if (C.use_tab == 2) hipLaunchKernelGGL((k_pair_emit2<2, true, true>), g, b, 0, st, B, F, C, seg_off, (uint32_t *)nullptr, keys, (void *)ids, 0u);
+    else if (C.use_tab) hipLaunchKernelGGL((k_pair_emit2<1, true, true>), g, b, 0, st, B, F, C, seg_off, (uint32_t *)nullptr, keys, (void *)ids, 0u);
+    else hipLaunchKernelGGL((k_pair_emit2<0, true, true>), g, b, 0, st, B, F, C, seg_off, (uint32_t *)nullptr, keys, (void *)ids, 0u);
 }
 void fd_launch_row_count(const fd_batch_view &B, const fd_hash_consts &C, uint32_t *row_cnt, float cutoff, hipStream_t st) {
     if (!B.n_work) return;
```
